# facebookresearch/rela

Hardware: AMD Instinct MI355X
Metric: env-steps/s (Ape-X Atari 84x84x4, actor tick + learner grad-step) (higher is better)
Workload: dtype f32 (f32 operands as 3 exact bf16 parts on bf16 MFMA; f32-accurate); 1 GPU; Ape-X DQN 80x80 envs/GPU, actor+learner on one MI355X, replay 2^20, B=512, A=18, n=3; device-resident static frames; parallelism=single

## Files before the change

### rela_amd/csrc/gemm_bf16x3.h

```cpp
#pragma once
#include <hip/hip_runtime.h>

#include <type_traits>

#include "common.h"
#include "gemm_lds.h"
#include "prof.h"

namespace rela_amd {
namespace gemm3 {

typedef float f32x4 __attribute__((ext_vector_type(4)));
typedef float f32x2 __attribute__((ext_vector_type(2)));
typedef __bf16 bf16x8 __attribute__((ext_vector_type(8)));
typedef __bf16 bf16x2 __attribute__((ext_vector_type(2)));
typedef short s16x4 __attribute__((ext_vector_type(4)));
typedef s16x4 __attribute__((address_space(3))) * lds_s16x4_ptr;

constexpr int kT = 512;
constexpr int BK = 32;

__device__ __forceinline__ int krow(int k) {
  const int g = k >> 3, j = k & 7;
  return j < 4 ? 4 * g + j : 16 + 4 * g + (j - 4);
}

__device__ __forceinline__ void split4(float4 v, uint2& hi, uint2& lo) {
  const f32x2 a = {v.x, v.y}, b = {v.z, v.w};
  const bf16x2 ha = __builtin_convertvector(a, bf16x2), hb = __builtin_convertvector(b, bf16x2);
  const bf16x2 la = __builtin_convertvector(a - __builtin_convertvector(ha, f32x2), bf16x2);
  const bf16x2 lb = __builtin_convertvector(b - __builtin_convertvector(hb, f32x2), bf16x2);
  hi = make_uint2(__builtin_bit_cast(uint32_t, ha), __builtin_bit_cast(uint32_t, hb));
  lo = make_uint2(__builtin_bit_cast(uint32_t, la), __builtin_bit_cast(uint32_t, lb));
}

__device__ __forceinline__ void split4x3(float4 v, uint2& hi, uint2& mid, uint2& lo) {
  const f32x2 a = {v.x, v.y}, b = {v.z, v.w};
  const bf16x2 ha = __builtin_convertvector(a, bf16x2), hb = __builtin_convertvector(b, bf16x2);
  const f32x2 ra = a - __builtin_convertvector(ha, f32x2), rb = b - __builtin_convertvector(hb, f32x2);
  const bf16x2 ma = __builtin_convertvector(ra, bf16x2), mb = __builtin_convertvector(rb, bf16x2);
  const bf16x2 la = __builtin_convertvector(ra - __builtin_convertvector(ma, f32x2), bf16x2);
  const bf16x2 lb = __builtin_convertvector(rb - __builtin_convertvector(mb, f32x2), bf16x2);
  hi = make_uint2(__builtin_bit_cast(uint32_t, ha), __builtin_bit_cast(uint32_t, hb));
  mid = make_uint2(__builtin_bit_cast(uint32_t, ma), __builtin_bit_cast(uint32_t, mb));
  lo = make_uint2(__builtin_bit_cast(uint32_t, la), __builtin_bit_cast(uint32_t, lb));
}

template <int BM_, int BN_, int WM_, int WN_, bool AMC_, int PARTS_ = 2>
struct TileCfg {
  static constexpr int BM = BM_, BN = BN_, WM = WM_, WN = WN_, PARTS = PARTS_;
  static constexpr bool AMC = AMC_;
  static_assert(PARTS == 2 || PARTS == 3, "two or three bf16 parts per operand");
  static_assert(WM * WN == 8, "8 wavefronts per block");
  static_assert(BM % 32 == 0 && BN % 32 == 0, "k-major row strides need multiples of 32 columns");
  static constexpr int TM = BM / 16 / WM, TN = BN / 16 / WN;
  static_assert(TM >= 1 && TN >= 1, "tile too small for the wave grid");
  static constexpr int LDA = AMC ? BM * 2 + 32 : BK * 2 + 16;
  static constexpr int A_HALF = AMC ? BK * LDA : BM * LDA;
  static constexpr int LDB = BN * 2 + 32;
  static constexpr int B_HALF = BK * LDB;
  static constexpr int BUF = PARTS * (A_HALF + B_HALF);
  static constexpr int LDS_BYTES = 2 * BUF;
  static constexpr int A_V4 = BM * BK / 4, B_V4 = BN * BK / 4;
  static constexpr int A_IT = (A_V4 + kT - 1) / kT, B_IT = (B_V4 + kT - 1) / kT;
};

struct GridMap {
  int gx, gy, gz;
  int mode;
};
__device__ __forceinline__ bool grid_map(const GridMap& gm, int& bx, int& by, int& bz) {
  if (gm.mode == 0) {
    bx = blockIdx.x, by = blockIdx.y, bz = blockIdx.z;
    return true;
  }
  const int xcd = blockIdx.x & 7, i = blockIdx.x >> 3;
  if (gm.mode == 1) {
    const int tiles = gm.gx * gm.gy;
    bz = (i / tiles) * 8 + xcd;
    const int t = i % tiles;
    bx = t % gm.gx, by = t / gm.gx;
    return bz < gm.gz;
  }
  bx = (i / gm.gy) * 8 + xcd, by = i % gm.gy, bz = 0;
  return bx < gm.gx;
}

template <class T, class P>
__global__ __launch_bounds__(kT) void gemm_bf16x3(const P p, const GridMap gm) {
  extern __shared__ __attribute__((aligned(16))) uint8_t smem[];
  int bx, by, bz;
  if (!grid_map(gm, bx, by, bz)) return;
  const int tid = threadIdx.x;
  const int wave = tid >> 6, lane = tid & 63;
  const int li = lane & 15, g = lane >> 4;
  const int wm = wave / T::WN, wn = wave % T::WN;
  const int m0 = by * T::BM, n0 = bx * T::BN;
  const int nch = (p.K + BK - 1) / BK;
  const int c0 = bz * p.kslice;
  const int c1 = min(nch, c0 + p.kslice);

  constexpr int D = 4;
  float4 ra[D][T::A_IT], rb[D][T::B_IT];
  auto gload = [&](int ch, auto set) {
    constexpr int S = decltype(set)::value;
    const int k0 = ch * BK;
#pragma unroll
    for (int j = 0; j < T::A_IT; ++j) {
      const int idx = min(tid + j * kT, T::A_V4 - 1);
      if constexpr (T::AMC) {
        const int kr = idx / (T::BM / 4), q = idx % (T::BM / 4);
        ra[S][j] = p.loadA(k0 + kr, m0 + 4 * q);
      } else {
        const int r = idx >> 3, q = idx & 7;
        ra[S][j] = p.loadA(m0 + r, k0 + 4 * q);
      }
    }
#pragma unroll
    for (int j = 0; j < T::B_IT; ++j) {
      const int idx = min(tid + j * kT, T::B_V4 - 1);
      const int kr = idx / (T::BN / 4), q = idx % (T::BN / 4);
      rb[S][j] = p.loadB(k0 + kr, n0 + 4 * q);
    }
  };
  auto sstore = [&](int buf, auto set) {
    constexpr int S = decltype(set)::value;
    uint8_t* base = smem + buf * T::BUF;
#pragma unroll
    for (int j = 0; j < T::A_IT; ++j) {
      const int idx = min(tid + j * kT, T::A_V4 - 1);
      uint2 hi, mid, lo;
      if constexpr (T::PARTS == 3) split4x3(ra[S][j], hi, mid, lo);
      else split4(ra[S][j], hi, lo);
      int off;
      if constexpr (T::AMC) {
        const int kr = idx / (T::BM / 4), q = idx % (T::BM / 4);
        off = krow(kr) * T::LDA + q * 8;
      } else {
        const int r = idx >> 3, q = idx & 7;
        off = r * T::LDA + q * 8;
      }
      *reinterpret_cast<uint2*>(base + off) = hi;
      if constexpr (T::PARTS == 3) *reinterpret_cast<uint2*>(base + T::A_HALF + off) = mid;
      *reinterpret_cast<uint2*>(base + (T::PARTS - 1) * T::A_HALF + off) = lo;
    }
    uint8_t* bb = base + T::PARTS * T::A_HALF;
#pragma unroll
    for (int j = 0; j < T::B_IT; ++j) {
      const int idx = min(tid + j * kT, T::B_V4 - 1);
      const int kr = idx / (T::BN / 4), q = idx % (T::BN / 4);
      uint2 hi, mid, lo;
      if constexpr (T::PARTS == 3) split4x3(rb[S][j], hi, mid, lo);
      else split4(rb[S][j], hi, lo);
      const int off = krow(kr) * T::LDB + q * 8;
      *reinterpret_cast<uint2*>(bb + off) = hi;
      if constexpr (T::PARTS == 3) *reinterpret_cast<uint2*>(bb + T::B_HALF + off) = mid;
      *reinterpret_cast<uint2*>(bb + (T::PARTS - 1) * T::B_HALF + off) = lo;
    }
  };

  const int tr_off = (4 * g + (li >> 2));
  auto frag_tr = [&](const uint8_t* img, int ld, int col0) -> bf16x8 {
    const uint8_t* a0 = img + tr_off * ld + (col0 + 4 * (li & 3)) * 2;
    const s16x4 x = __builtin_amdgcn_ds_read_tr16_b64_v4i16((lds_s16x4_ptr)(a0));
    const s16x4 y = __builtin_amdgcn_ds_read_tr16_b64_v4i16((lds_s16x4_ptr)(a0 + 16 * ld));
    typedef short s16x8 __attribute__((ext_vector_type(8)));
    const s16x8 z = {x[0], x[1], x[2], x[3], y[0], y[1], y[2], y[3]};
    return __builtin_bit_cast(bf16x8, z);
  };
  auto frag_row = [&](const uint8_t* img, int row) -> bf16x8 {
    return __builtin_bit_cast(bf16x8, *reinterpret_cast<const uint4*>(img + row * T::LDA + g * 16));
  };

  f32x4 acc[T::TM][T::TN];
  f32x4 accs[T::PARTS == 3 ? T::TM : 1][T::PARTS == 3 ? T::TN : 1];
#pragma unroll
  for (int t = 0; t < T::TM; ++t)
#pragma unroll
    for (int u = 0; u < T::TN; ++u) {
      acc[t][u] = f32x4{0.f, 0.f, 0.f, 0.f};
      if constexpr (T::PARTS == 3) accs[t][u] = f32x4{0.f, 0.f, 0.f, 0.f};
    }

  using S0 = std::integral_constant<int, 0>;
  using S1 = std::integral_constant<int, 1>;
  using S2 = std::integral_constant<int, 2>;
  using S3 = std::integral_constant<int, 3>;
  if (c0 < c1) gload(c0, S0{});
  if (c0 + 1 < c1) gload(c0 + 1, S1{});
  if (c0 + 2 < c1) gload(c0 + 2, S2{});
  if (c0 + 3 < c1) gload(c0 + 3, S3{});
  if (c0 < c1) sstore(0, S0{});
  __syncthreads();
  auto step = [&](int cur, auto cs, auto ns) {
    const int buf = (cur - c0) & 1;
    if (cur + D < c1) gload(cur + D, cs);
    const uint8_t* base = smem + buf * T::BUF;
    const uint8_t* bb = base + T::PARTS * T::A_HALF;
    bf16x8 bp[T::TN][T::PARTS];
#pragma unroll
    for (int u = 0; u < T::TN; ++u) {
      const int col0 = (wn * T::TN + u) * 16;
#pragma unroll
      for (int q = 0; q < T::PARTS; ++q) bp[u][q] = frag_tr(bb + q * T::B_HALF, T::LDB, col0);
    }
#pragma unroll
    for (int t = 0; t < T::TM; ++t) {
      const int row0 = (wm * T::TM + t) * 16;
      bf16x8 ap[T::PARTS];
#pragma unroll
      for (int q = 0; q < T::PARTS; ++q) {
        if constexpr (T::AMC) ap[q] = frag_tr(base + q * T::A_HALF, T::LDA, row0);
        else ap[q] = frag_row(base + q * T::A_HALF, row0 + li);
      }
#pragma unroll
      for (int u = 0; u < T::TN; ++u) {
        if constexpr (T::PARTS == 2) {
          acc[t][u] = __builtin_amdgcn_mfma_f32_16x16x32_bf16(ap[1], bp[u][0], acc[t][u], 0, 0, 0);
          acc[t][u] = __builtin_amdgcn_mfma_f32_16x16x32_bf16(ap[0], bp[u][1], acc[t][u], 0, 0, 0);
          acc[t][u] = __builtin_amdgcn_mfma_f32_16x16x32_bf16(ap[0], bp[u][0], acc[t][u], 0, 0, 0);
        } else {
          accs[t][u] = __builtin_amdgcn_mfma_f32_16x16x32_bf16(ap[2], bp[u][0], accs[t][u], 0, 0, 0);
          accs[t][u] = __builtin_amdgcn_mfma_f32_16x16x32_bf16(ap[0], bp[u][2], accs[t][u], 0, 0, 0);
          accs[t][u] = __builtin_amdgcn_mfma_f32_16x16x32_bf16(ap[1], bp[u][1], accs[t][u], 0, 0, 0);
          accs[t][u] = __builtin_amdgcn_mfma_f32_16x16x32_bf16(ap[1], bp[u][0], accs[t][u], 0, 0, 0);
          accs[t][u] = __builtin_amdgcn_mfma_f32_16x16x32_bf16(ap[0], bp[u][1], accs[t][u], 0, 0, 0);
          acc[t][u] = __builtin_amdgcn_mfma_f32_16x16x32_bf16(ap[0], bp[u][0], acc[t][u], 0, 0, 0);
        }
      }
    }
    if (cur + 1 < c1) sstore(buf ^ 1, ns);
    __syncthreads();
  };
  for (int base = c0; base < c1; base += D) {
    step(base, S0{}, S1{});
    if (base + 1 < c1) step(base + 1, S1{}, S2{});
    if (base + 2 < c1) step(base + 2, S2{}, S3{});
    if (base + 3 < c1) step(base + 3, S3{}, S0{});
  }

#pragma unroll
  for (int t = 0; t < T::TM; ++t)
#pragma unroll
    for (int u = 0; u < T::TN; ++u)
#pragma unroll
      for (int r = 0; r < 4; ++r) {
        const int m = m0 + (wm * T::TM + t) * 16 + g * 4 + r;
        const int n = n0 + (wn * T::TN + u) * 16 + li;
        if (m < p.M && n < p.N) {
          if constexpr (T::PARTS == 3) p.store(bz, m, n, acc[t][u][r] + accs[t][u][r]);
          else p.store(bz, m, n, acc[t][u][r]);
        }
      }
}

template <class T, class P>
int launch_gemm(P p, int splits, hipStream_t s, const char* name) {
  static const hipError_t attr_set = hipFuncSetAttribute(reinterpret_cast<const void*>(&gemm_bf16x3<T, P>),
                                                         hipFuncAttributeMaxDynamicSharedMemorySize, T::LDS_BYTES);
  RELA_HIP(attr_set);
  const int nch = ceil_div(p.K, BK);
  p.kslice = ceil_div(nch, splits);
  ProfScope prof(name, s);
  note_launch("gemm_bf16x3");
  constexpr bool xmap = true;
  GridMap gm{ceil_div(p.N, T::BN), ceil_div(p.M, T::BM), splits, 0};
  dim3 grid(gm.gx, gm.gy, gm.gz);
  if (xmap && gm.gz >= 8) {
    gm.mode = 1;
    grid = dim3(8 * gm.gx * gm.gy * ceil_div(gm.gz, 8));
  } else if (xmap && gm.gz == 1 && gm.gy > 1 && gm.gx >= 8) {
    gm.mode = 2;
    grid = dim3(8 * gm.gy * ceil_div(gm.gx, 8));
  }
  hipLaunchKernelGGL((gemm_bf16x3<T, P>), grid, dim3(kT), T::LDS_BYTES, s, p, gm);
  return RELA_OK;
}

}
}
```

### rela_amd/csrc/gemm_lds.h

```cpp
#pragma once
#include <hip/hip_runtime.h>

#include "common.h"
#include "prof.h"

namespace rela_amd {
namespace gemm {

typedef float f32x4 __attribute__((ext_vector_type(4)));
constexpr int kLT = 512;
constexpr int BK = 32;

__device__ __forceinline__ float4 zero4() { return make_float4(0.f, 0.f, 0.f, 0.f); }
__device__ __forceinline__ float4 ld4(const float* p) { return *reinterpret_cast<const float4*>(p); }

template <int BM_, int BN_, int WM_, int WN_, bool AMC_>
struct TileCfg {
  static constexpr int BM = BM_, BN = BN_, WM = WM_, WN = WN_;
  static constexpr bool AMC = AMC_;
  static_assert(WM * WN == 8, "8 wavefronts per block");
  static constexpr int TM = BM / 16 / WM, TN = BN / 16 / WN;
  static_assert(TM >= 1 && TN >= 1, "tile too small for the wave grid");
  static constexpr int LDA = AMC ? BM + 16 : BK + 2;
  static constexpr int A_FLOATS = AMC ? BK * LDA : BM * LDA;
  static constexpr int LDB = BN + 16;
  static constexpr int B_FLOATS = BK * LDB;
  static constexpr int A_V4 = BM * BK / 4, B_V4 = BN * BK / 4;
  static constexpr int A_IT = (A_V4 + kLT - 1) / kLT, B_IT = (B_V4 + kLT - 1) / kLT;
};

template <class T, class P>
__global__ __launch_bounds__(kLT) void gemm_lds(const P p) {
  __shared__ __attribute__((aligned(16))) float sA[2][T::A_FLOATS];
  __shared__ __attribute__((aligned(16))) float sB[2][T::B_FLOATS];
  const int tid = threadIdx.x;
  const int wave = tid >> 6, lane = tid & 63;
  const int li = lane & 15, kk = lane >> 4;
  const int wm = wave / T::WN, wn = wave % T::WN;
  const int m0 = blockIdx.y * T::BM, n0 = blockIdx.x * T::BN;
  const int nch = (p.K + BK - 1) / BK;
  const int c0 = blockIdx.z * p.kslice;
  const int c1 = min(nch, c0 + p.kslice);

  float4 ra[T::A_IT], rb[T::B_IT];
  auto gload = [&](int ch) {
    const int k0 = ch * BK;
#pragma unroll
    for (int j = 0; j < T::A_IT; ++j) {
      const int idx = tid + j * kLT;
      if (idx < T::A_V4) {
        if constexpr (T::AMC) {
          const int kr = idx / (T::BM / 4), q = idx % (T::BM / 4);
          ra[j] = p.loadA(k0 + kr, m0 + 4 * q);
        } else {
          const int r = idx >> 3, q = idx & 7;
          ra[j] = p.loadA(m0 + r, k0 + 4 * q);
        }
      }
    }
#pragma unroll
    for (int j = 0; j < T::B_IT; ++j) {
      const int idx = tid + j * kLT;
      if (idx < T::B_V4) {
        const int kr = idx / (T::BN / 4), q = idx % (T::BN / 4);
        rb[j] = p.loadB(k0 + kr, n0 + 4 * q);
      }
    }
  };
  auto sstore = [&](int buf) {
#pragma unroll
    for (int j = 0; j < T::A_IT; ++j) {
      const int idx = tid + j * kLT;
      if (idx < T::A_V4) {
        if constexpr (T::AMC) {
          const int kr = idx / (T::BM / 4), q = idx % (T::BM / 4);
          *reinterpret_cast<float4*>(&sA[buf][kr * T::LDA + 4 * q]) = ra[j];
        } else {
          const int r = idx >> 3, q = idx & 7;
          float* d = &sA[buf][r * T::LDA + 4 * q];
          *reinterpret_cast<float2*>(d) = make_float2(ra[j].x, ra[j].y);
          *reinterpret_cast<float2*>(d + 2) = make_float2(ra[j].z, ra[j].w);
        }
      }
    }
#pragma unroll
    for (int j = 0; j < T::B_IT; ++j) {
      const int idx = tid + j * kLT;
      if (idx < T::B_V4) {
        const int kr = idx / (T::BN / 4), q = idx % (T::BN / 4);
        *reinterpret_cast<float4*>(&sB[buf][kr * T::LDB + 4 * q]) = rb[j];
      }
    }
  };

  f32x4 acc[T::TM][T::TN];
#pragma unroll
  for (int t = 0; t < T::TM; ++t)
#pragma unroll
    for (int u = 0; u < T::TN; ++u) acc[t][u] = f32x4{0.f, 0.f, 0.f, 0.f};

  if (c0 < c1) {
    gload(c0);
    sstore(0);
  }
  __syncthreads();
  for (int ch = c0; ch < c1; ++ch) {
    const int buf = (ch - c0) & 1;
    if (ch + 1 < c1) gload(ch + 1);
#pragma unroll
    for (int ks = 0; ks < BK / 4; ++ks) {
      float a[T::TM], b[T::TN];
#pragma unroll
      for (int t = 0; t < T::TM; ++t) {
        const int row = (wm * T::TM + t) * 16 + li;
        a[t] = T::AMC ? sA[buf][(4 * ks + kk) * T::LDA + row] : sA[buf][row * T::LDA + 4 * ks + kk];
      }
#pragma unroll
      for (int u = 0; u < T::TN; ++u) b[u] = sB[buf][(4 * ks + kk) * T::LDB + (wn * T::TN + u) * 16 + li];
#pragma unroll
      for (int t = 0; t < T::TM; ++t)
#pragma unroll
        for (int u = 0; u < T::TN; ++u) acc[t][u] = __builtin_amdgcn_mfma_f32_16x16x4f32(a[t], b[u], acc[t][u], 0, 0, 0);
    }
    if (ch + 1 < c1) sstore(buf ^ 1);
    __syncthreads();
  }

#pragma unroll
  for (int t = 0; t < T::TM; ++t)
#pragma unroll
    for (int u = 0; u < T::TN; ++u)
#pragma unroll
      for (int r = 0; r < 4; ++r) {
        const int m = m0 + (wm * T::TM + t) * 16 + kk * 4 + r;
        const int n = n0 + (wn * T::TN + u) * 16 + li;
        if (m < p.M && n < p.N) p.store(blockIdx.z, m, n, acc[t][u][r]);
      }
}

struct ProbBase {
  int M, N, K, kslice;
};

template <class T, class P>
void launch_gemm(P p, int splits, hipStream_t s, const char* name) {
  const int nch = ceil_div(p.K, BK);
  p.kslice = ceil_div(nch, splits);
  ProfScope prof(name, s);
  note_launch("gemm_lds (f32)");
  hipLaunchKernelGGL((gemm_lds<T, P>), dim3(ceil_div(p.N, T::BN), ceil_div(p.M, T::BM), splits), dim3(kLT), 0, s, p);
}

}
}
```

### rela_amd/csrc/learner.hip

```cpp
#include "learner_common.h"

using namespace rela_amd;

struct rela_apex_learner {
  int device = 0;
  int A = 0, Bmax = 0;
  float gamma_n = 0.f;
  float vr_eps = 0.f;
  bool loss_called = false;
  int optimizer = 0;
  float lr = 0.f, opt_eps = 0.f, clip = 0.f;
  int64_t adam_t = 0;
  int64_t off[13] = {0};
  float *P = nullptr, *PT = nullptr, *G = nullptr, *S1 = nullptr, *S2 = nullptr;
  rela_ffnet *online = nullptr, *target = nullptr;
  float *w2p = nullptr, *w3p = nullptr, *wfcp = nullptr;
  void *ws_on = nullptr, *ws_tmp = nullptr;
  int64_t ws_bytes = 0;
  float *q = nullptr;
  float *td = nullptr, *d_ha = nullptr, *d_h = nullptr, *d_a3 = nullptr, *d_a2 = nullptr, *d_a1 = nullptr;
  float *col = nullptr;
  float *part = nullptr;
  float *cpart = nullptr;
  float *s32 = nullptr;
  double* npart = nullptr;
  float* norm = nullptr;
  float* loss = nullptr;
  bool loaded = false;
  int pend_B = 0, last_B = 0;
  int pend_rows = 0;
  const uint8_t* pend_obs = nullptr;
  hipStream_t side = nullptr;
  hipEvent_t ev[8] = {nullptr};
  float *part_side = nullptr, *cpart_side = nullptr;
  void *frag2 = nullptr, *frag3 = nullptr;
};

namespace {
rela_ffnet_params params_at(const rela_apex_learner* l, float* base) {
  rela_ffnet_params p;
  const float** f = reinterpret_cast<const float**>(&p);
  for (int i = 0; i < 12; ++i) f[i] = base + l->off[i];
  return p;
}

int repack(rela_apex_learner* l, bool online, bool target, hipStream_t s) {
  if (online) {
    const rela_ffnet_params p = params_at(l, l->P);
    FFNetExtraPacks extra;
    extra.w2p = l->w2p, extra.w3p = l->w3p, extra.wfcp = l->wfcp;
    int rc = ffnet_load_extra(l->online, &p, s, extra);
    if (rc != RELA_OK) return rc;
    if (l->frag2) dgfast::pack_frags(l->w2p, l->w3p, l->frag2, l->frag3, s);
  }
  if (target) {
    const rela_ffnet_params p = params_at(l, l->PT);
    int rc = rela_ffnet_load(l->target, &p, 1, s);
    if (rc != RELA_OK) return rc;
  }
  return RELA_OK;
}
}

extern "C" int rela_apex_learner_create(rela_apex_learner** out, int num_action, int max_batch, int multi_step,
                                        float gamma, int optimizer, float lr, float eps, float grad_clip,
                                        int device) {
  RELA_CHECK(out && num_action >= 1 && num_action <= 31 && max_batch >= 1 && multi_step >= 1 &&
                 (optimizer == 0 || optimizer == 1),
             RELA_EINVAL, "rela_apex_learner_create: bad arguments (A=%d batch=%d n=%d optimizer=%d)", num_action,
             max_batch, multi_step, optimizer);
  int ndev = 0;
  if (hipGetDeviceCount(&ndev) != hipSuccess || device < 0 || device >= ndev) {
    set_last_error("rela_apex_learner_create: HIP device %d not available (%d visible); there is no CPU path",
                   device, ndev);
    return RELA_ENODEV;
  }
  DeviceGuard g(device);
  auto* l = new rela_apex_learner();
  l->device = device;
  l->A = num_action;
  l->Bmax = max_batch;
  l->gamma_n = (float)pow((double)gamma, (double)multi_step);
  l->optimizer = optimizer;
  l->lr = lr;
  l->opt_eps = eps;
  l->clip = grad_clip;
  const int64_t cnt[12] = {32 * 256, 32, 64 * 512, 64, 64 * 576, 64, (int64_t)512 * 3136, 512, 512, 1,
                           (int64_t)num_action * 512, num_action};
  for (int i = 0; i < 12; ++i) l->off[i + 1] = l->off[i] + (cnt[i] + 3) / 4 * 4;
  const size_t nb = sizeof(float) * (size_t)l->off[12];
  const size_t B = (size_t)max_batch, A = (size_t)num_action;
  RELA_HIP(hipMalloc(&l->P, nb));
  RELA_HIP(hipMalloc(&l->PT, nb));
  RELA_HIP(hipMalloc(&l->G, nb));
  RELA_HIP(hipMalloc(&l->S1, nb));
  RELA_HIP(hipMalloc(&l->S2, nb));
  RELA_HIP(hipMemset(l->P, 0, nb));
  RELA_HIP(hipMemset(l->PT, 0, nb));
  RELA_HIP(hipMemset(l->G, 0, nb));
  RELA_HIP(hipMemset(l->S1, 0, nb));
  RELA_HIP(hipMemset(l->S2, 0, nb));
  int rc = rela_ffnet_create(&l->online, num_action, device);
  if (rc != RELA_OK) return rc;
  rc = rela_ffnet_create(&l->target, num_action, device);
  if (rc != RELA_OK) return rc;
  ffnet_label_as_learner(l->online);
  ffnet_label_as_learner(l->target);
  ffnet_set_max_rows(l->online, max_batch);
  ffnet_set_max_rows(l->target, max_batch);
  RELA_HIP(hipMalloc(&l->w2p, sizeof(float) * 64 * 512));
  RELA_HIP(hipMalloc(&l->w3p, sizeof(float) * 64 * 576));
  RELA_HIP(hipMalloc(&l->wfcp, sizeof(float) * 512 * 3136));
  l->ws_bytes = std::max(rela_ffnet_workspace_bytes(nullptr, max_batch), rela_ffnet_workspace_bytes(nullptr, 2 * max_batch));
  RELA_HIP(hipMalloc(&l->ws_on, (size_t)l->ws_bytes));
  RELA_HIP(hipMalloc(&l->ws_tmp, (size_t)l->ws_bytes));
  RELA_HIP(hipMalloc(&l->q, sizeof(float) * 3 * B * A));
  RELA_HIP(hipMalloc(&l->td, sizeof(float) * B));
  RELA_HIP(hipMalloc(&l->d_ha, sizeof(float) * B * 32));
  RELA_HIP(hipMalloc(&l->d_h, sizeof(float) * B * 512));
  RELA_HIP(hipMalloc(&l->d_a3, sizeof(float) * B * kA3));
  RELA_HIP(hipMalloc(&l->d_a2, sizeof(float) * B * kA2));
  RELA_HIP(hipMalloc(&l->d_a1, sizeof(float) * B * kA1));
  RELA_HIP(hipMalloc(&l->col, sizeof(float) * trunk_col_floats(B)));
  RELA_HIP(hipMalloc(&l->part, sizeof(float) * kTrunkPartFloats));
  RELA_HIP(hipMalloc(&l->cpart, sizeof(float) * kColsumBlocks * (32 + 512 + 64 + 64 + 32)));
  RELA_HIP(hipMalloc(&l->s32, sizeof(float) * 32));
  RELA_HIP(hipMalloc(&l->npart, sizeof(double) * kNormBlocks));
  RELA_HIP(hipMalloc(&l->norm, sizeof(float) * 2));
  RELA_HIP(hipMalloc(&l->loss, sizeof(float)));
  static const bool lanes = !(getenv("RELA_LEARNER_LANES") && atoi(getenv("RELA_LEARNER_LANES")) == 1);
  if (lanes) {
    RELA_HIP(hipStreamCreateWithFlags(&l->side, hipStreamNonBlocking));
    for (hipEvent_t& e : l->ev) RELA_HIP(hipEventCreateWithFlags(&e, hipEventDisableTiming));
    RELA_HIP(hipMalloc(&l->part_side, sizeof(float) * kTrunkPartFloats));
    RELA_HIP(hipMalloc(&l->cpart_side, sizeof(float) * kColsumBlocks * (32 + 512 + 64 + 64 + 32)));
    RELA_HIP(hipMalloc(&l->frag2, dgfast::kFrag2Bytes));
    RELA_HIP(hipMalloc(&l->frag3, dgfast::kFrag3Bytes));
  }
  *out = l;
  return RELA_OK;
}

extern "C" void rela_apex_learner_destroy(rela_apex_learner* l) {
  if (!l) return;
  DeviceGuard g(l->device);
  (void)hipDeviceSynchronize();
  void* ps[] = {l->P,  l->PT,   l->G,    l->S1,   l->S2,   l->w2p, l->w3p,  l->wfcp,  l->ws_on, l->ws_tmp, l->q,
                l->td, l->d_ha, l->d_h,  l->d_a3, l->d_a2, l->d_a1, l->col, l->part,  l->cpart, l->s32,    l->npart,
                l->norm, l->loss, l->part_side, l->cpart_side, l->frag2, l->frag3};
  for (void* p : ps) (void)hipFree(p);
  for (hipEvent_t e : l->ev)
    if (e) (void)hipEventDestroy(e);
  if (l->side) (void)hipStreamDestroy(l->side);
  rela_ffnet_destroy(l->online);
  rela_ffnet_destroy(l->target);
  delete l;
}

extern "C" int rela_apex_learner_load(rela_apex_learner* l, const rela_ffnet_params* online,
                                      const rela_ffnet_params* target, int on_device, void* stream_) {
  RELA_CHECK(l && online, RELA_EINVAL, "rela_apex_learner_load: bad arguments");
  hipStream_t s = (hipStream_t)stream_;
  DeviceGuard g(l->device);
  const hipMemcpyKind kind = on_device ? hipMemcpyDeviceToDevice : hipMemcpyHostToDevice;
  const float* const* fo = reinterpret_cast<const float* const*>(online);
  const float* const* ft = reinterpret_cast<const float* const*>(target ? target : online);
  const int64_t cnt[12] = {32 * 256, 32, 64 * 512, 64, 64 * 576, 64, (int64_t)512 * 3136, 512, 512, 1,
                           (int64_t)l->A * 512, l->A};
  for (int i = 0; i < 12; ++i) {
    RELA_CHECK(fo[i] && ft[i], RELA_EINVAL, "rela_apex_learner_load: parameter %d is NULL", i);
    RELA_HIP(hipMemcpyAsync(l->P + l->off[i], fo[i], sizeof(float) * cnt[i], kind, s));
    RELA_HIP(hipMemcpyAsync(l->PT + l->off[i], ft[i], sizeof(float) * cnt[i], kind, s));
  }
  if (!on_device) RELA_HIP(hipStreamSynchronize(s));
  const size_t nb = sizeof(float) * (size_t)l->off[12];
  RELA_HIP(hipMemsetAsync(l->S1, 0, nb, s));
  RELA_HIP(hipMemsetAsync(l->S2, 0, nb, s));
  l->adam_t = 0;
  int rc = repack(l, true, true, s);
  if (rc != RELA_OK) return rc;
  l->loaded = true;
  return RELA_OK;
}

extern "C" int rela_apex_learner_set_value_rescale(rela_apex_learner* l, float eps) {
  RELA_CHECK(l && eps == eps, RELA_EINVAL, "rela_apex_learner_set_value_rescale: bad arguments");
  RELA_CHECK(!l->loss_called, RELA_ESTATE, "rela_apex_learner_set_value_rescale: call it before the first loss");
  l->vr_eps = eps > 0.f ? eps : 0.f;
  return RELA_OK;
}

extern "C" int rela_apex_learner_set_precision(rela_apex_learner* l, int mode) {
  RELA_CHECK(l && mode >= 0 && mode <= 2, RELA_EINVAL, "rela_apex_learner_set_precision: mode must be 0, 1 or 2");
  int rc = rela_ffnet_set_precision(l->online, mode);
  if (rc != RELA_OK) return rc;
  return rela_ffnet_set_precision(l->target, mode);
}

extern "C" int rela_apex_learner_sync_target(rela_apex_learner* l, void* stream_) {
  RELA_CHECK(l && l->loaded, RELA_ESTATE, "rela_apex_learner_sync_target: parameters were never loaded");
  hipStream_t s = (hipStream_t)stream_;
  DeviceGuard g(l->device);
  RELA_HIP(hipMemcpyAsync(l->PT, l->P, sizeof(float) * (size_t)l->off[12], hipMemcpyDeviceToDevice, s));
  return repack(l, false, true, s);
}

extern "C" int rela_apex_learner_params(rela_apex_learner* l, rela_ffnet_params* online_out,
                                        rela_ffnet_params* target_out) {
  RELA_CHECK(l, RELA_EINVAL, "rela_apex_learner_params: bad arguments");
  if (online_out) *online_out = params_at(l, l->P);
  if (target_out) *target_out = params_at(l, l->PT);
  return RELA_OK;
}

extern "C" int rela_apex_learner_grads(rela_apex_learner* l, rela_ffnet_params* grads_out) {
  RELA_CHECK(l && grads_out, RELA_EINVAL, "rela_apex_learner_grads: bad arguments");
  *grads_out = params_at(l, l->G);
  return RELA_OK;
}

extern "C" int rela_apex_learner_flat(rela_apex_learner* l, float** params_dev, float** grads_dev, int64_t* count) {
  RELA_CHECK(l, RELA_EINVAL, "rela_apex_learner_flat: bad arguments");
  if (params_dev) *params_dev = l->P;
  if (grads_dev) *grads_dev = l->G;
  if (count) *count = l->off[12];
  return RELA_OK;
}

extern "C" const float* rela_apex_learner_stats_dev(const rela_apex_learner* l) { return l ? l->norm : nullptr; }

extern "C" int rela_apex_learner_debug_activations(rela_apex_learner* l, float** a1, float** a2, float** a3, float** h,
                                                   int* batch) {
  RELA_CHECK(l && l->last_B > 0, RELA_ESTATE, "rela_apex_learner_debug_activations: no rela_apex_learner_loss yet");
  const FFNetWs w = ffnet_ws(l->ws_on, l->pend_rows);
  if (a1) *a1 = w.a1;
  if (a2) *a2 = w.a2;
  if (a3) *a3 = w.a3;
  if (h) *h = w.h;
  if (batch) *batch = l->last_B;
  return RELA_OK;
}

extern "C" int rela_apex_learner_backward(rela_apex_learner* l, int batch, const void* const* rows_dev,
                                          const float* weight_dev, float* priority_dev, float* loss_dev,
                                          void* stream_) {
  int rc = rela_apex_learner_loss(l, batch, rows_dev, weight_dev, priority_dev, loss_dev, stream_);
  if (rc != RELA_OK) return rc;
  return rela_apex_learner_grad(l, stream_);
}

static bool merge_online_forwards() {
  static const bool on = [] {
    const char* e = getenv("RELA_LEARNER_MERGE_ONLINE");
    return !(e && e[0] == '0');
  }();
  return on;
}

extern "C" int rela_apex_learner_loss(rela_apex_learner* l, int batch, const void* const* rows_dev,
                                      const float* weight_dev, float* priority_dev, float* loss_dev, void* stream_) {
  RELA_CHECK(l && l->loaded, RELA_ESTATE, "rela_apex_learner_loss: parameters were never loaded");
  RELA_CHECK(batch >= 1 && batch <= l->Bmax && rows_dev && weight_dev && priority_dev, RELA_EINVAL,
             "rela_apex_learner_loss: bad arguments (batch %d, max %d)", batch, l->Bmax);
  l->pend_B = 0;
  l->loss_called = true;
  hipStream_t s = (hipStream_t)stream_;
  DeviceGuard g(l->device);
  const int Bn = batch, A = l->A;
  const uint8_t* obs = static_cast<const uint8_t*>(rows_dev[0]);
  const uint8_t* nobs = static_cast<const uint8_t*>(rows_dev[1]);
  const float* legal = static_cast<const float*>(rows_dev[4]);
  const float* nlegal = static_cast<const float*>(rows_dev[5]);
  const int64_t* act = static_cast<const int64_t*>(rows_dev[6]);
  const float* reward = static_cast<const float*>(rows_dev[7]);
  const float* boot = static_cast<const float*>(rows_dev[9]);
  RELA_CHECK(obs && nobs && legal && nlegal && act && reward && boot, RELA_EINVAL,
             "rela_apex_learner_loss: a batch field is NULL");
  float* q_on = l->q;
  float* q_no = l->q + (size_t)Bn * A;
  float* q_nt = l->q + 2 * (size_t)Bn * A;
  int rc;
  bool unsplit_side = false;
  l->pend_rows = Bn;
  if (rela_ffnet_precision(l->online) == 1 && ffnet_learner_forward_ok(l->online, l->target, Bn)) {
    rc = ffnet_learner_forward(l->online, l->target, Bn, obs, nobs, legal, nlegal, q_on, q_no, q_nt, l->ws_on, l->ws_tmp,
                               l->ws_bytes, s);
    if (rc != RELA_OK) return rc;
    if (l->side) lane_dep(l->ev[0], s, l->side);
    rc = ffnet_learner_unsplit(Bn, l->ws_on, l->side ? l->side : s);
    if (rc != RELA_OK) return rc;
    unsplit_side = l->side != nullptr;
    l->pend_rows = 2 * Bn;
  } else if (rela_ffnet_precision(l->online) == 2 && Bn >= 512 && merge_online_forwards() &&
             nobs == obs + (size_t)Bn * 28224 && nlegal == legal + (size_t)Bn * A) {
    const uint8_t* in2 = obs;
    const float* legal2 = legal;
    rc = rela_ffnet_forward(l->target, Bn, nobs, nlegal, q_nt, l->ws_tmp, l->ws_bytes, s);
    if (rc != RELA_OK) return rc;
    ffnet_set_max_rows(l->online, 2 * l->Bmax);
    rc = ffnet_forward_mode(l->online, 2 * Bn, in2, legal2, q_on, l->ws_on, l->ws_bytes, s, 3);
    ffnet_set_max_rows(l->online, l->Bmax);
    if (rc != RELA_OK) return rc;
    l->pend_rows = 2 * Bn;
  } else {
    rc = rela_ffnet_forward(l->online, Bn, nobs, nlegal, q_no, l->ws_tmp, l->ws_bytes, s);
    if (rc != RELA_OK) return rc;
    rc = rela_ffnet_forward(l->target, Bn, nobs, nlegal, q_nt, l->ws_tmp, l->ws_bytes, s);
    if (rc != RELA_OK) return rc;
    rc = ffnet_forward_mode(l->online, Bn, obs, legal, q_on, l->ws_on, l->ws_bytes, s, rela_ffnet_precision(l->online) == 2 ? 3 : 0);
    if (rc != RELA_OK) return rc;
  }
  if (Bn <= 1024) {
    ProfScope prof("learner_loss_grad", s);
    hipLaunchKernelGGL(learner_td_loss_grad, dim3(1), dim3(1024), 0, s, Bn, A, (const float*)q_on, (const float*)q_no,
                       (const float*)q_nt, nlegal, act, reward, boot, l->gamma_n, l->vr_eps, weight_dev, legal, l->td,
                       priority_dev, l->d_ha, l->loss);
  } else {
    rc = td_from_q(Bn, A, 0, q_on, q_no, q_nt, nlegal, act, reward, boot, l->gamma_n, l->vr_eps, l->td, priority_dev, s);
    if (rc != RELA_OK) return rc;
    ProfScope prof("learner_loss_grad", s);
    hipLaunchKernelGGL(learner_loss_grad, dim3(1), dim3(kLT), 0, s, (const float*)l->td, weight_dev, act, legal, Bn,
                       A, l->d_ha, l->loss);
  }
  if (loss_dev) RELA_HIP(dev_copy2(loss_dev, l->loss, sizeof(float), nullptr, nullptr, 0, s));
  if (unsplit_side) lane_dep(l->ev[1], l->side, s);
  RELA_LAUNCH_CHECK();
  l->pend_B = l->last_B = Bn;
  l->pend_obs = obs;
  return RELA_OK;
}

extern "C" int rela_apex_learner_grad(rela_apex_learner* l, void* stream_) {
  RELA_CHECK(l && l->loaded && l->pend_B > 0, RELA_ESTATE, "rela_apex_learner_grad: no rela_apex_learner_loss to differentiate");
  hipStream_t s = (hipStream_t)stream_;
  DeviceGuard g(l->device);
  const int Bn = l->pend_B, A = l->A;
  const uint8_t* obs = l->pend_obs;
  l->pend_B = 0;

  const FFNetWs w = ffnet_ws(l->ws_on, l->pend_rows);
  const rela_ffnet_params P = params_at(l, l->P);
  float* Gm[12];
  for (int i = 0; i < 12; ++i) Gm[i] = l->G + l->off[i];

  ColsumJobs sums;
  const bool g3 = rela_ffnet_precision(l->online) == 1 && gemm_bf16x3_on();
  const bool g6 = rela_ffnet_precision(l->online) == 2;
  const bool lanes = l->side != nullptr;
  hipStream_t sw = lanes ? l->side : s;
  if (lanes) lane_dep(l->ev[2], s, sw);

  {
    ProbHeadDgrad p{};
    p.M = Bn, p.N = 512, p.K = 32;
    p.d_ha = l->d_ha, p.a_w = P.a_w, p.v_w = P.v_w, p.h = w.h, p.d_h = l->d_h, p.A = A;
    if (g3) (void)gemm3::launch_gemm<Tile3Dgrad>(p, 1, s, "learner_dgrad_heads");
    else if (g6) (void)gemm3::launch_gemm<Tile6Dgrad>(p, 1, s, "learner_dgrad_heads");
    else launch_gemm<TileDgrad>(p, 1, s, "learner_dgrad_heads");
  }
  {
    ProbHeadWgrad p{};
    p.M = 32, p.N = 512, p.K = Bn;
    p.d_ha = l->d_ha, p.h = w.h, p.g_a_w = Gm[10], p.g_v_w = Gm[8], p.A = A;
    if (g3) (void)gemm3::launch_gemm<Tile3W32>(p, 1, sw, "learner_wgrad_heads");
    else if (g6) (void)gemm3::launch_gemm<Tile6W32>(p, 1, sw, "learner_wgrad_heads");
    else launch_gemm<TileW32>(p, 1, sw, "learner_wgrad_heads");
  }
  sums.add(l->d_ha, Bn, 32, l->s32);
  if (lanes) lane_dep(l->ev[3], s, sw);
  {
    ProbFcDgrad p{};
    p.M = Bn, p.N = 3136, p.K = 512;
    p.d_h = l->d_h, p.wfcp = l->wfcp, p.a3 = w.a3, p.d_a3 = l->d_a3;
    if (g3) (void)gemm3::launch_gemm<Tile3Dgrad>(p, 1, s, "learner_dgrad_fc");
    else if (g6) (void)gemm3::launch_gemm<Tile6Dgrad>(p, 1, s, "learner_dgrad_fc");
    else launch_gemm<TileDgrad>(p, 1, s, "learner_dgrad_fc");
  }
  {
    ProbFcWgrad p{};
    p.M = 512, p.N = 3136, p.K = Bn;
    p.d_h = l->d_h, p.a3 = w.a3, p.g_fc_w = Gm[6];
    if (g3) (void)gemm3::launch_gemm<Tile3Wfc>(p, 1, sw, "learner_wgrad_fc");
    else if (g6) (void)gemm3::launch_gemm<Tile6Wfc>(p, 1, sw, "learner_wgrad_fc");
    else launch_gemm<TileWfc>(p, 1, sw, "learner_wgrad_fc");
  }
  sums.add(l->d_h, Bn, 512, Gm[7]);
  {
    TrunkBwd t{};
    t.Bn = Bn, t.obs = obs, t.a1 = w.a1, t.a2 = w.a2, t.d_a3 = l->d_a3, t.d_a2 = l->d_a2, t.d_a1 = l->d_a1;
    t.col = l->col, t.part = l->part, t.cpart = l->cpart, t.w2p = l->w2p, t.w3p = l->w3p;
    t.g_c1w = Gm[0], t.g_c1b = Gm[1], t.g_c2w = Gm[2], t.g_c2b = Gm[3], t.g_c3w = Gm[4], t.g_c3b = Gm[5];
    t.fast = rela_ffnet_precision(l->online) == 1;
    t.emu = g6;
    if (lanes) {
      t.side = sw, t.ev_da3 = l->ev[4], t.ev_da2 = l->ev[5], t.ev_side = l->ev[6];
      t.part_side = l->part_side, t.cpart_side = l->cpart_side;
      if (t.fast) t.frag2 = l->frag2, t.frag3 = l->frag3;
      t.s32 = l->s32, t.A = A, t.g_a_b = Gm[11], t.g_v_b = Gm[9];
    }
    trunk_backward(t, s, &sums);
    if (!lanes) hipLaunchKernelGGL(head_bias_grad, dim3(1), dim3(32), 0, s, (const float*)l->s32, A, Gm[11], Gm[9]);
  }
  RELA_LAUNCH_CHECK();
  return RELA_OK;
}

namespace {
struct TrunkTapScratch {
  std::vector<void*> bufs;
  hipStream_t side = nullptr;
  hipEvent_t ev[3] = {nullptr, nullptr, nullptr};
  ~TrunkTapScratch() {
    for (void* p : bufs) (void)hipFree(p);
    for (hipEvent_t e : ev)
      if (e) (void)hipEventDestroy(e);
    if (side) (void)hipStreamDestroy(side);
  }
  template <class T>
  hipError_t alloc(T** p, size_t bytes) {
    void* v = nullptr;
    const hipError_t e = hipMalloc(&v, bytes);
    if (e == hipSuccess) bufs.push_back(v);
    *p = static_cast<T*>(v);
    return e;
  }
};
}

extern "C" int rela_debug_trunk_backward(int frames, int mode, int lanes, int fast_wgrad_min_frames, const uint8_t* obs,
                                         const float* a1, const float* a2, const float* d_a3, const float* conv2_w,
                                         const float* conv3_w, float* g_c1w, float* g_c1b, float* g_c2w, float* g_c2b,
                                         float* g_c3w, float* g_c3b, float* d_a2, float* d_a1, void* stream_) {
  RELA_CHECK(frames >= 1 && frames <= 65536 && mode >= 0 && mode <= 2 && (lanes == 0 || lanes == 1), RELA_EINVAL,
             "rela_debug_trunk_backward: bad arguments (frames %d, mode %d, lanes %d)", frames, mode, lanes);
  RELA_CHECK(obs && a1 && a2 && d_a3 && conv2_w && conv3_w && g_c1w && g_c1b && g_c2w && g_c2b && g_c3w && g_c3b && d_a2 &&
                 d_a1,
             RELA_EINVAL, "rela_debug_trunk_backward: a pointer is NULL");
  hipStream_t s = (hipStream_t)stream_;
  TrunkTapScratch sc;
  const size_t cpart_bytes = sizeof(float) * kColsumBlocks * (32 + 512 + 64 + 64 + 32);
  float *w2p = nullptr, *w3p = nullptr;
  RELA_HIP(sc.alloc(&w2p, sizeof(float) * 64 * 512));
  RELA_HIP(sc.alloc(&w3p, sizeof(float) * 64 * 576));
  hipLaunchKernelGGL(permute_weights, dim3(ceil_div(64 * 512, 256)), dim3(256), 0, s, kPermConv2, conv2_w, w2p, 64 * 512);
  hipLaunchKernelGGL(permute_weights, dim3(ceil_div(64 * 576, 256)), dim3(256), 0, s, kPermConv3, conv3_w, w3p, 64 * 576);
  TrunkBwd t{};
  t.Bn = frames, t.obs = obs, t.a1 = a1, t.a2 = a2, t.d_a3 = d_a3, t.d_a2 = d_a2, t.d_a1 = d_a1;
  t.w2p = w2p, t.w3p = w3p;
  t.g_c1w = g_c1w, t.g_c1b = g_c1b, t.g_c2w = g_c2w, t.g_c2b = g_c2b, t.g_c3w = g_c3w, t.g_c3b = g_c3b;
  t.fast = mode == 1;
  if (fast_wgrad_min_frames > 0) t.fast_wgrad_min_frames = fast_wgrad_min_frames;
  RELA_HIP(sc.alloc(&t.col, sizeof(float) * trunk_col_floats((size_t)frames)));
  RELA_HIP(sc.alloc(&t.part, sizeof(float) * kTrunkPartFloats));
  RELA_HIP(sc.alloc(&t.cpart, cpart_bytes));
  t.emu = mode == 2;
  if (lanes) {
    RELA_HIP(hipStreamCreateWithFlags(&sc.side, hipStreamNonBlocking));
    for (hipEvent_t& e : sc.ev) RELA_HIP(hipEventCreateWithFlags(&e, hipEventDisableTiming));
    t.side = sc.side, t.ev_da3 = sc.ev[0], t.ev_da2 = sc.ev[1], t.ev_side = sc.ev[2];
    RELA_HIP(sc.alloc(&t.part_side, sizeof(float) * kTrunkPartFloats));
    RELA_HIP(sc.alloc(&t.cpart_side, cpart_bytes));
    if (t.fast) {
      void *frag2 = nullptr, *frag3 = nullptr;
      RELA_HIP(sc.alloc(&frag2, dgfast::kFrag2Bytes));
      RELA_HIP(sc.alloc(&frag3, dgfast::kFrag3Bytes));
      dgfast::pack_frags(w2p, w3p, frag2, frag3, s);
      t.frag2 = frag2, t.frag3 = frag3;
    }
  }
  trunk_backward(t, s);
  const hipError_t launched = hipGetLastError();
  const hipError_t done = hipStreamSynchronize(s);
  if (sc.side) (void)hipStreamSynchronize(sc.side);
  RELA_HIP(launched);
  RELA_HIP(done);
  return RELA_OK;
}

extern "C" int rela_apex_learner_apply(rela_apex_learner* l, void* stream_) {
  RELA_CHECK(l && l->loaded, RELA_ESTATE, "rela_apex_learner_apply: parameters were never loaded");
  hipStream_t s = (hipStream_t)stream_;
  DeviceGuard g(l->device);
  OptimState o;
  o.optimizer = l->optimizer, o.lr = l->lr, o.eps = l->opt_eps, o.clip = l->clip, o.adam_t = l->adam_t;
  optimizer_apply(o, l->P, l->G, l->S1, l->S2, l->off[12], l->npart, l->norm, s);
  l->adam_t = o.adam_t;
  RELA_LAUNCH_CHECK();
  return repack(l, true, false, s);
}
```

### rela_amd/csrc/learner_common.h

```cpp
#pragma once
#include <cmath>
#include <cstring>
#include <vector>

#include "common.h"
#include "ffnet_layout.h"
#include "gemm_lds.h"
#include "gemm_bf16x3.h"
#include "prof.h"
#include "value_rescale.h"
#include "dgrad_conv_bf16.h"
#include "wgrad_conv1_bf16.h"
#include "wgrad_conv2_bf16.h"
#include "wgrad_conv3_bf16.h"

namespace rela_amd {
namespace {

using namespace gemm;

using TileDgrad = TileCfg<128, 64, 4, 2, false>;
using TileWfc = TileCfg<128, 64, 4, 2, true>;
using TileW64 = TileCfg<64, 64, 2, 4, true>;
using TileW32 = TileCfg<32, 64, 2, 4, true>;
using Tile3Dgrad = gemm3::TileCfg<128, 64, 4, 2, false>;
using Tile3Wfc = gemm3::TileCfg<128, 64, 4, 2, true>;
using Tile3W64 = gemm3::TileCfg<64, 64, 2, 4, true>;
using Tile3W32 = gemm3::TileCfg<32, 64, 2, 4, true>;
inline bool gemm_bf16x3_on() { return true; }
using Tile6Dgrad = gemm3::TileCfg<128, 64, 4, 2, false, 3>;
using Tile6Wfc = gemm3::TileCfg<128, 64, 4, 2, true, 3>;
using Tile6W64 = gemm3::TileCfg<64, 64, 2, 4, true, 3>;
using Tile6W32 = gemm3::TileCfg<32, 64, 2, 4, true, 3>;


struct ProbHeadDgrad : ProbBase {
  const float *d_ha, *a_w, *v_w, *h;
  float* d_h;
  int A;
  __device__ float4 loadA(int m, int k) const { return m < M ? ld4(d_ha + (size_t)m * 32 + k) : zero4(); }
  __device__ float4 loadB(int k, int n) const {
    if (k < A) return ld4(a_w + (size_t)k * 512 + n);
    if (k == 31) return ld4(v_w + n);
    return zero4();
  }
  __device__ void store(int, int m, int n, float v) const {
    const size_t i = (size_t)m * 512 + n;
    d_h[i] = h[i] > 0.f ? v : 0.f;
  }
};

struct ProbHeadWgradPart : ProbBase {
  const float *d_ha, *h;
  float* part;
  __device__ float4 loadA(int b, int m) const { return b < K ? ld4(d_ha + (size_t)b * 32 + m) : zero4(); }
  __device__ float4 loadB(int b, int n) const { return b < K ? ld4(h + (size_t)b * 512 + n) : zero4(); }
  __device__ void store(int z, int m, int n, float v) const { part[((size_t)z * 32 + m) * 512 + n] = v; }
};
__global__ void head_wgrad_reduce(const float* __restrict__ part, int splits, int A, float* __restrict__ g_a_w,
                                  float* __restrict__ g_v_w) {
  const int idx = blockIdx.x * blockDim.x + threadIdx.x;
  if (idx >= 32 * 512) return;
  const int m = idx >> 9, n = idx & 511;
  if (m >= A && m != 31) return;
  float s = 0.f;
#pragma unroll 8
  for (int z = 0; z < splits; ++z) s += part[(size_t)z * (32 * 512) + idx];
  if (m < A) g_a_w[(size_t)m * 512 + n] = s;
  else g_v_w[n] = s;
}

struct ProbHeadWgrad : ProbBase {
  const float *d_ha, *h;
  float *g_a_w, *g_v_w;
  int A;
  __device__ float4 loadA(int b, int m) const { return b < K ? ld4(d_ha + (size_t)b * 32 + m) : zero4(); }
  __device__ float4 loadB(int b, int n) const { return b < K ? ld4(h + (size_t)b * 512 + n) : zero4(); }
  __device__ void store(int, int m, int n, float v) const {
    if (m < A) g_a_w[(size_t)m * 512 + n] = v;
    else if (m == 31) g_v_w[n] = v;
  }
};

struct ProbFcDgrad : ProbBase {
  const float *d_h, *wfcp, *a3;
  float* d_a3;
  __device__ float4 loadA(int m, int k) const { return m < M ? ld4(d_h + (size_t)m * 512 + k) : zero4(); }
  __device__ float4 loadB(int k, int n) const { return ld4(wfcp + (size_t)k * 3136 + n); }
  __device__ void store(int, int m, int n, float v) const {
    const size_t i = (size_t)m * 3136 + n;
    d_a3[i] = a3[i] > 0.f ? v : 0.f;
  }
};

struct ProbFcWgrad : ProbBase {
  const float *d_h, *a3;
  float* g_fc_w;
  __device__ float4 loadA(int b, int m) const { return b < K ? ld4(d_h + (size_t)b * 512 + m) : zero4(); }
  __device__ float4 loadB(int b, int n) const { return b < K ? ld4(a3 + (size_t)b * 3136 + n) : zero4(); }
  __device__ void store(int, int m, int n, float v) const {
    const int pos = n >> 6, c = n & 63;
    g_fc_w[(size_t)m * 3136 + c * 49 + pos] = v;
  }
};

struct ProbConvDgrad : ProbBase {
  const float *d_out, *wp;
  float* col;
  __device__ float4 loadA(int m, int k) const { return m < M ? ld4(d_out + (size_t)m * 64 + k) : zero4(); }
  __device__ float4 loadB(int k, int n) const { return ld4(wp + (size_t)k * N + n); }
  __device__ void store(int, int m, int n, float v) const { col[(size_t)m * N + n] = v; }
};

template <int OC, int CIN, int KH, int KW, int STRIDE, int OH, int OW, int IH, int IW>
struct ProbConvWgrad : ProbBase {
  const float *d_out, *in;
  float* part;
  __device__ float4 loadA(int k, int m) const { return k < K ? ld4(d_out + (size_t)k * OC + m) : zero4(); }
  __device__ float4 loadB(int k, int n) const {
    if (k >= K) return zero4();
    const int b = k / (OH * OW), pos = k - b * (OH * OW);
    const int oy = pos / OW, ox = pos - oy * OW;
    const int r = n / CIN, c = n - r * CIN;
    const int kh = r / KW, kw = r - kh * KW;
    return ld4(in + (((size_t)b * IH + oy * STRIDE + kh) * IW + ox * STRIDE + kw) * CIN + c);
  }
  __device__ void store(int z, int m, int n, float v) const { part[((size_t)z * M + m) * N + n] = v; }
};
using ProbW3 = ProbConvWgrad<64, 64, 3, 3, 1, 7, 7, 9, 9>;
using ProbW2 = ProbConvWgrad<64, 32, 4, 4, 2, 9, 9, 20, 20>;

struct ProbW1 : ProbBase {
  const float* d_out;
  const uint8_t* obs;
  float* part;
  __device__ float4 loadA(int k, int m) const { return k < K ? ld4(d_out + (size_t)k * 32 + m) : zero4(); }
  __device__ float4 loadB(int k, int n) const {
    if (k >= K) return zero4();
    const int b = k / 400, pos = k - b * 400;
    const int oy = pos / 20, ox = pos - oy * 20;
    const int c = n >> 6, kh = (n >> 3) & 7, kw = n & 7;
    const uint32_t d = *reinterpret_cast<const uint32_t*>(obs + (size_t)b * 28224 + c * 7056 + (oy * 4 + kh) * 84 +
                                                          ox * 4 + kw);
    return make_float4((float)(d & 0xff), (float)((d >> 8) & 0xff), (float)((d >> 16) & 0xff), (float)(d >> 24));
  }
  __device__ void store(int z, int m, int n, float v) const { part[((size_t)z * M + m) * N + n] = v; }
};


__global__ void col2im3(const float* __restrict__ col, const float* __restrict__ a2, float* __restrict__ d_a2,
                        int Bn) {
  const int idx = blockIdx.x * blockDim.x + threadIdx.x;
  if (idx >= Bn * 81 * 16) return;
  const int c4 = idx & 15, pix = idx >> 4;
  const int x = pix % 9, y = (pix / 9) % 9, b = pix / 81;
  float4 s = zero4();
  for (int kh = 0; kh < 3; ++kh) {
    const int oy = y - kh;
    if (oy < 0 || oy >= 7) continue;
    for (int kw = 0; kw < 3; ++kw) {
      const int ox = x - kw;
      if (ox < 0 || ox >= 7) continue;
      const float4 v = ld4(col + ((size_t)b * 49 + oy * 7 + ox) * 576 + (kh * 3 + kw) * 64 + c4 * 4);
      s.x += v.x, s.y += v.y, s.z += v.z, s.w += v.w;
    }
  }
  const float4 a = ld4(a2 + (size_t)pix * 64 + c4 * 4);
  *reinterpret_cast<float4*>(d_a2 + (size_t)pix * 64 + c4 * 4) =
      make_float4(a.x > 0.f ? s.x : 0.f, a.y > 0.f ? s.y : 0.f, a.z > 0.f ? s.z : 0.f, a.w > 0.f ? s.w : 0.f);
}

__global__ void col2im2(const float* __restrict__ col, const float* __restrict__ a1, float* __restrict__ d_a1,
                        int Bn) {
  const int idx = blockIdx.x * blockDim.x + threadIdx.x;
  if (idx >= Bn * 400 * 8) return;
  const int c4 = idx & 7, pix = idx >> 3;
  const int x = pix % 20, y = (pix / 20) % 20, b = pix / 400;
  float4 s = zero4();
  for (int kh = 0; kh < 4; ++kh) {
    const int ty = y - kh;
    if (ty < 0 || (ty & 1) || ty > 16) continue;
    for (int kw = 0; kw < 4; ++kw) {
      const int tx = x - kw;
      if (tx < 0 || (tx & 1) || tx > 16) continue;
      const float4 v = ld4(col + ((size_t)b * 81 + (ty >> 1) * 9 + (tx >> 1)) * 512 + (kh * 4 + kw) * 32 + c4 * 4);
      s.x += v.x, s.y += v.y, s.z += v.z, s.w += v.w;
    }
  }
  const float4 a = ld4(a1 + (size_t)pix * 32 + c4 * 4);
  *reinterpret_cast<float4*>(d_a1 + (size_t)pix * 32 + c4 * 4) =
      make_float4(a.x > 0.f ? s.x : 0.f, a.y > 0.f ? s.y : 0.f, a.z > 0.f ? s.z : 0.f, a.w > 0.f ? s.w : 0.f);
}

enum { kRedConv1 = 0, kRedConv2 = 1, kRedConv3 = 2 };
__global__ void reduce_splits(const float* __restrict__ part, int splits, int M, int N, int mode,
                              float* __restrict__ out) {
  const int idx = blockIdx.x * blockDim.x + threadIdx.x;
  if (idx >= M * N) return;
  const int m = idx / N, n = idx - m * N;
  float s = 0.f;
#pragma unroll 8
  for (int z = 0; z < splits; ++z) s += part[((size_t)z * M + m) * N + n];
  if (mode == kRedConv1) {
    out[(size_t)m * N + n] = s / 255.0f;
  } else if (mode == kRedConv2) {
    const int c = n & 31, r = n >> 5;
    out[((size_t)(m * 32 + c) * 4 + (r >> 2)) * 4 + (r & 3)] = s;
  } else {
    const int c = n & 63, r = n >> 6;
    out[((size_t)(m * 64 + c) * 3 + r / 3) * 3 + r % 3] = s;
  }
}

constexpr int kColsumBlocks = 256;
__global__ __launch_bounds__(kLT) void colsum_partial(const float* __restrict__ src, int64_t rows, int C,
                                                      float* __restrict__ part) {
  __shared__ float4 sm[kLT];
  const int G = C / 4, L = kLT / G;
  const int cg = threadIdx.x % G, rl = threadIdx.x / G;
  const int64_t per = (rows + gridDim.x - 1) / gridDim.x;
  const int64_t r0 = blockIdx.x * per, r1 = min(rows, r0 + per);
  float4 s = zero4();
  for (int64_t r = r0 + rl; r < r1; r += L) {
    const float4 v = ld4(src + r * C + cg * 4);
    s.x += v.x, s.y += v.y, s.z += v.z, s.w += v.w;
  }
  sm[threadIdx.x] = s;
  __syncthreads();
  if (rl == 0) {
    for (int l = 1; l < L; ++l) {
      const float4 v = sm[cg + l * G];
      s.x += v.x, s.y += v.y, s.z += v.z, s.w += v.w;
    }
    *reinterpret_cast<float4*>(part + (size_t)blockIdx.x * C + cg * 4) = s;
  }
}
__global__ __launch_bounds__(kColsumBlocks) void colsum_final(const float* __restrict__ part, int C,
                                                              float* __restrict__ out) {
  __shared__ float4 sm[kColsumBlocks];
  const int cg = blockIdx.x;
  sm[threadIdx.x] = ld4(part + (size_t)threadIdx.x * C + cg * 4);
  __syncthreads();
  for (int o = kColsumBlocks / 2; o > 0; o >>= 1) {
    if ((int)threadIdx.x < o) {
      const float4 v = sm[threadIdx.x + o];
      float4& d = sm[threadIdx.x];
      d.x += v.x, d.y += v.y, d.z += v.z, d.w += v.w;
    }
    __syncthreads();
  }
  if (threadIdx.x == 0) *reinterpret_cast<float4*>(out + cg * 4) = sm[0];
}
constexpr int kMaxColsumJobs = 6;
struct ColsumJobs {
  const float* src[kMaxColsumJobs];
  float* out[kMaxColsumJobs];
  float* part[kMaxColsumJobs];
  int64_t rows[kMaxColsumJobs];
  int C[kMaxColsumJobs];
  int n = 0;
  void add(const float* s, int64_t r, int c, float* o) { src[n] = s, rows[n] = r, C[n] = c, out[n] = o, ++n; }
};
__global__ __launch_bounds__(kLT) void colsum_partial_multi(ColsumJobs jobs) {
  __shared__ float4 sm[kLT];
  const int j = blockIdx.y;
  const float* src = jobs.src[j];
  const int64_t rows = jobs.rows[j];
  const int C = jobs.C[j];
  const int G = C / 4, L = kLT / G;
  const int cg = threadIdx.x % G, rl = threadIdx.x / G;
  const int64_t per = (rows + gridDim.x - 1) / gridDim.x;
  const int64_t r0 = blockIdx.x * per, r1 = min(rows, r0 + per);
  float4 s = zero4();
  int64_t r = r0 + rl;
  for (; r + 7 * (int64_t)L < r1; r += 8 * (int64_t)L) {
    float4 v[8];
#pragma unroll
    for (int u = 0; u < 8; ++u) v[u] = ld4(src + (r + u * (int64_t)L) * C + cg * 4);
#pragma unroll
    for (int u = 0; u < 8; ++u) s.x += v[u].x, s.y += v[u].y, s.z += v[u].z, s.w += v[u].w;
  }
  for (; r < r1; r += L) {
    const float4 v = ld4(src + r * C + cg * 4);
    s.x += v.x, s.y += v.y, s.z += v.z, s.w += v.w;
  }
  sm[threadIdx.x] = s;
  __syncthreads();
  if (rl == 0) {
    for (int l = 1; l < L; ++l) {
      const float4 v = sm[cg + l * G];
      s.x += v.x, s.y += v.y, s.z += v.z, s.w += v.w;
    }
    *reinterpret_cast<float4*>(jobs.part[j] + (size_t)blockIdx.x * C + cg * 4) = s;
  }
}
__global__ __launch_bounds__(kColsumBlocks) void colsum_final_multi(ColsumJobs jobs) {
  __shared__ float4 sm[kColsumBlocks];
  const int j = blockIdx.y, cg = blockIdx.x, C = jobs.C[j];
  if (cg >= C / 4) return;
  sm[threadIdx.x] = ld4(jobs.part[j] + (size_t)threadIdx.x * C + cg * 4);
  __syncthreads();
  for (int o = kColsumBlocks / 2; o > 0; o >>= 1) {
    if ((int)threadIdx.x < o) {
      const float4 v = sm[threadIdx.x + o];
      float4& d = sm[threadIdx.x];
      d.x += v.x, d.y += v.y, d.z += v.z, d.w += v.w;
    }
    __syncthreads();
  }
  if (threadIdx.x == 0) *reinterpret_cast<float4*>(jobs.out[j] + cg * 4) = sm[0];
}
__global__ void head_bias_grad(const float* __restrict__ s32, int A, float* __restrict__ g_a_b,
                               float* __restrict__ g_v_b) {
  const int k = threadIdx.x;
  if (k < A) g_a_b[k] = s32[k];
  if (k == 31) g_v_b[0] = s32[31];
}

__global__ __launch_bounds__(kLT) void learner_loss_grad(const float* __restrict__ td, const float* __restrict__ w,
                                                         const int64_t* __restrict__ act,
                                                         const float* __restrict__ legal, int Bn, int A,
                                                         float* __restrict__ d_ha, float* __restrict__ loss_out) {
  __shared__ float red[kLT];
  float lsum = 0.f;
  const float inv_b = 1.0f / (float)Bn, inv_a = 1.0f / (float)A;
  for (int i = threadIdx.x; i < Bn; i += kLT) {
    const float e = td[i], ae = fabsf(e);
    lsum += (ae < 1.0f ? 0.5f * e * e : ae - 0.5f) * w[i];
    const float g = -(w[i] * fminf(fmaxf(e, -1.0f), 1.0f)) * inv_b;
    const int a = (int)act[i];
    float* row = d_ha + (size_t)i * 32;
    for (int k = 0; k < 32; ++k) {
      float v = 0.f;
      if (k < A) v = legal[(size_t)i * A + k] * (g * ((k == a ? 1.0f : 0.0f) - inv_a));
      if (k == 31) v = g;
      row[k] = v;
    }
  }
  red[threadIdx.x] = lsum;
  __syncthreads();
  for (int o = kLT / 2; o > 0; o >>= 1) {
    if (threadIdx.x < o) red[threadIdx.x] += red[threadIdx.x + o];
    __syncthreads();
  }
  if (threadIdx.x == 0) loss_out[0] = red[0] * inv_b;
}

__global__ __launch_bounds__(1024) void learner_td_loss_grad(int Bn, int A, const float* __restrict__ q,
                                                             const float* __restrict__ qno, const float* __restrict__ qnt,
                                                             const float* __restrict__ nlegal,
                                                             const int64_t* __restrict__ act,
                                                             const float* __restrict__ reward,
                                                             const float* __restrict__ bootstrap, float gamma_n,
                                                             float vr_eps, const float* __restrict__ w,
                                                             const float* __restrict__ legal,
                                                             float* __restrict__ td, float* __restrict__ prio,
                                                             float* __restrict__ d_ha, float* __restrict__ loss_out) {
  __shared__ float red[1024];
  float m = INFINITY;
  for (int i = threadIdx.x; i < Bn * A; i += 1024) m = fminf(m, qno[i]);
  red[threadIdx.x] = m;
  __syncthreads();
  for (int off = 512; off > 0; off >>= 1) {
    if ((int)threadIdx.x < off) red[threadIdx.x] = fminf(red[threadIdx.x], red[threadIdx.x + off]);
    __syncthreads();
  }
  const float qmin = red[0];
  __syncthreads();
  float lsum = 0.f;
  const float inv_b = 1.0f / (float)Bn, inv_a = 1.0f / (float)A;
  for (int i = threadIdx.x; i < Bn; i += 1024) {
    int na = 0;
    float bv = -INFINITY;
#pragma unroll 6
    for (int j = 0; j < A; ++j) {
      const float lq = __fmul_rn(__fsub_rn(__fadd_rn(1.0f, qno[(size_t)i * A + j]), qmin), nlegal[(size_t)i * A + j]);
      if (lq > bv) bv = lq, na = j;
    }
    const int a = (int)act[i];
    const float qa = q[(size_t)i * A + a];
    const float bq = qnt[(size_t)i * A + na];
    float tgt;
    if (vr_eps > 0.0f)
      tgt = rela_vr::h(__fadd_rn(reward[i], __fmul_rn(__fmul_rn(bootstrap[i], gamma_n), rela_vr::h_inv(bq, vr_eps))), vr_eps);
    else
      tgt = __fadd_rn(reward[i], __fmul_rn(__fmul_rn(bootstrap[i], gamma_n), bq));
    const float e = __fsub_rn(tgt, qa), ae = fabsf(e);
    td[i] = e;
    prio[i] = ae;
    lsum += (ae < 1.0f ? 0.5f * e * e : ae - 0.5f) * w[i];
    const float g = -(w[i] * fminf(fmaxf(e, -1.0f), 1.0f)) * inv_b;
    float4* row = reinterpret_cast<float4*>(d_ha + (size_t)i * 32);
    float v[32];
#pragma unroll
    for (int k = 0; k < 32; ++k) {
      v[k] = 0.f;
      if (k < A) v[k] = legal[(size_t)i * A + k] * (g * ((k == a ? 1.0f : 0.0f) - inv_a));
      if (k == 31) v[k] = g;
    }
#pragma unroll
    for (int k = 0; k < 8; ++k) row[k] = make_float4(v[4 * k], v[4 * k + 1], v[4 * k + 2], v[4 * k + 3]);
  }
  red[threadIdx.x] = lsum;
  __syncthreads();
  for (int o = 512; o > 0; o >>= 1) {
    if ((int)threadIdx.x < o) red[threadIdx.x] += red[threadIdx.x + o];
    __syncthreads();
  }
  if (threadIdx.x == 0) loss_out[0] = red[0] * inv_b;
}

__global__ void permute_weights(int mode, const float* __restrict__ src, float* __restrict__ dst, int total) {
  const int idx = blockIdx.x * blockDim.x + threadIdx.x;
  if (idx < total) permute_weight_at(mode, idx, src, dst);
}

constexpr int kNormBlocks = 256;
__global__ __launch_bounds__(256) void sumsq_partial(const float* __restrict__ g, int64_t n, double* __restrict__ part) {
  __shared__ double red[256];
  double s = 0.0;
  const int64_t n4 = n >> 2, stride = (int64_t)gridDim.x * 256;
  const float4* g4 = reinterpret_cast<const float4*>(g);
  int64_t i = (int64_t)blockIdx.x * 256 + threadIdx.x;
  for (; i + 3 * stride < n4; i += 4 * stride) {
    float4 v[4];
#pragma unroll
    for (int u = 0; u < 4; ++u) v[u] = g4[i + u * stride];
#pragma unroll
    for (int u = 0; u < 4; ++u)
      s += (double)v[u].x * (double)v[u].x + (double)v[u].y * (double)v[u].y + (double)v[u].z * (double)v[u].z +
           (double)v[u].w * (double)v[u].w;
  }
  for (; i < n4; i += stride) {
    const float4 v = g4[i];
    s += (double)v.x * (double)v.x + (double)v.y * (double)v.y + (double)v.z * (double)v.z + (double)v.w * (double)v.w;
  }
  if (blockIdx.x == 0 && threadIdx.x < (n & 3)) s += (double)g[(n4 << 2) + threadIdx.x] * (double)g[(n4 << 2) + threadIdx.x];
  red[threadIdx.x] = s;
  __syncthreads();
  for (int o = 128; o > 0; o >>= 1) {
    if (threadIdx.x < o) red[threadIdx.x] += red[threadIdx.x + o];
    __syncthreads();
  }
  if (threadIdx.x == 0) part[blockIdx.x] = red[0];
}
__global__ __launch_bounds__(256) void clip_coef(const double* __restrict__ part, int nblk, float max_norm,
                                                 float* __restrict__ out, const unsigned* __restrict__ abort_word) {
  __shared__ double red[256];
  red[threadIdx.x] = (int)threadIdx.x < nblk ? part[threadIdx.x] : 0.0;
  __syncthreads();
  for (int o = 128; o > 0; o >>= 1) {
    if ((int)threadIdx.x < o) red[threadIdx.x] += red[threadIdx.x + o];
    __syncthreads();
  }
  if (threadIdx.x != 0) return;
  const double s = red[0];
  const float norm = (float)sqrt(s);
  out[0] = norm;
  const float c = max_norm / (norm + 1e-6f);
  out[1] = c < 1.0f ? c : 1.0f;
  if (abort_word && *abort_word != 0) out[1] = -1.0f;
}
__global__ void rmsprop_update(float* __restrict__ p, const float* __restrict__ g, float* __restrict__ sq, int64_t n4,
                               float lr, float alpha, float eps, const float* __restrict__ coef) {
  const int64_t i = (int64_t)blockIdx.x * blockDim.x + threadIdx.x;
  const float cf = coef[1];
  if (i >= n4 || cf < 0.f) return;
  const float4 gv = reinterpret_cast<const float4*>(g)[i];
  float4 sv = reinterpret_cast<float4*>(sq)[i], pv = reinterpret_cast<float4*>(p)[i];
  auto upd = [&](float gi, float& s, float& pi) {
    gi = gi * cf;
    s = alpha * s + (1.0f - alpha) * gi * gi;
    pi -= lr * (gi / (sqrtf(s) + eps));
  };
  upd(gv.x, sv.x, pv.x), upd(gv.y, sv.y, pv.y), upd(gv.z, sv.z, pv.z), upd(gv.w, sv.w, pv.w);
  reinterpret_cast<float4*>(sq)[i] = sv;
  reinterpret_cast<float4*>(p)[i] = pv;
}
__global__ void adam_update(float* __restrict__ p, const float* __restrict__ g, float* __restrict__ m1,
                            float* __restrict__ m2, int64_t n4, float lr, float b1, float b2, float eps, float bc1,
                            float bc2_sqrt, const float* __restrict__ coef) {
  const int64_t i = (int64_t)blockIdx.x * blockDim.x + threadIdx.x;
  const float cf = coef[1];
  if (i >= n4 || cf < 0.f) return;
  const float4 gv = reinterpret_cast<const float4*>(g)[i];
  float4 av = reinterpret_cast<float4*>(m1)[i], bv = reinterpret_cast<float4*>(m2)[i], pv = reinterpret_cast<float4*>(p)[i];
  auto upd = [&](float gi, float& a, float& b, float& pi) {
    gi = gi * cf;
    a = b1 * a + (1.0f - b1) * gi;
    b = b2 * b + (1.0f - b2) * gi * gi;
    pi -= (lr / bc1) * (a / (sqrtf(b) / bc2_sqrt + eps));
  };
  upd(gv.x, av.x, bv.x, pv.x), upd(gv.y, av.y, bv.y, pv.y), upd(gv.z, av.z, bv.z, pv.z), upd(gv.w, av.w, bv.w, pv.w);
  reinterpret_cast<float4*>(m1)[i] = av;
  reinterpret_cast<float4*>(m2)[i] = bv;
  reinterpret_cast<float4*>(p)[i] = pv;
}


constexpr int kSplitW3 = 28, kSplitW2 = 27, kSplitW1 = 64;
constexpr size_t kTrunkPartFloats = (size_t)w3fast::kMaxBlocks * 64 * 576;
static_assert(kTrunkPartFloats * 4 >= dgfast::kFrag3Bytes && kTrunkPartFloats * 4 >= dgfast::kFrag2Bytes, "frag scratch");
static_assert(kTrunkPartFloats >= (size_t)kSplitW3 * 8 * 64 * 576, "part size (split multiplier up to 8)");
static_assert(kTrunkPartFloats >= (size_t)kSplitW3 * 64 * 576 && kTrunkPartFloats >= (size_t)w1fast::kMaxBlocks * 32 * 256 &&
                  kTrunkPartFloats >= (size_t)w2fast::kMaxBlocks * 64 * 512,
              "part size");
static_assert(kSplitW3 * 64 * 576 >= kSplitW2 * 64 * 512 && kSplitW3 * 64 * 576 >= kSplitW1 * 32 * 256, "part size");
inline size_t trunk_col_floats(size_t frames) { return frames * (size_t)(81 * 512 > 49 * 576 ? 81 * 512 : 49 * 576); }

constexpr int kFastWgradMinFrames = 2048;
struct TrunkBwd {
  int Bn;
  const uint8_t* obs;
  const float *a1, *a2;
  const float* d_a3;
  float *d_a2, *d_a1;
  float* col;
  float* part;
  float* cpart;
  const float *w2p, *w3p;
  float *g_c1w, *g_c1b, *g_c2w, *g_c2b, *g_c3w, *g_c3b;
  bool fast = false;
  bool emu = false;
  int fast_wgrad_min_frames = kFastWgradMinFrames;
  hipStream_t side = nullptr;
  hipEvent_t ev_da3 = nullptr, ev_da2 = nullptr, ev_side = nullptr;
  float *part_side = nullptr, *cpart_side = nullptr;
  const void *frag2 = nullptr, *frag3 = nullptr;
  const float* s32 = nullptr;
  float *g_a_b = nullptr, *g_v_b = nullptr;
  int A = 0;
};
inline void lane_dep(hipEvent_t ev, hipStream_t from, hipStream_t to) {
  (void)hipEventRecord(ev, from);
  (void)hipStreamWaitEvent(to, ev, 0);
}

inline void colsum_multi_launch(ColsumJobs& jobs, float* cpart, hipStream_t s) {
  if (jobs.n == 0) return;
  int maxC = 0;
  size_t off = 0;
  for (int j = 0; j < jobs.n; ++j) {
    jobs.part[j] = cpart + off;
    off += (size_t)kColsumBlocks * jobs.C[j];
    maxC = jobs.C[j] > maxC ? jobs.C[j] : maxC;
  }
  ProfScope prof("learner_colsum", s);
  hipLaunchKernelGGL(colsum_partial_multi, dim3(kColsumBlocks, jobs.n), dim3(kLT), 0, s, jobs);
  hipLaunchKernelGGL(colsum_final_multi, dim3(maxC / 4, jobs.n), dim3(kColsumBlocks), 0, s, jobs);
}

inline void colsum_launch(const float* src, int64_t rows, int C, float* cpart, float* out, hipStream_t s) {
  ProfScope prof("learner_colsum", s);
  hipLaunchKernelGGL(colsum_partial, dim3(kColsumBlocks), dim3(kLT), 0, s, src, rows, C, cpart);
  hipLaunchKernelGGL(colsum_final, dim3(C / 4), dim3(kColsumBlocks), 0, s, (const float*)cpart, C, out);
}

inline void trunk_backward(const TrunkBwd& t, hipStream_t s, ColsumJobs* pending = nullptr) {
  const int Bn = t.Bn;
  ColsumJobs own;
  ColsumJobs& jobs = pending ? *pending : own;
  const bool lanes = t.side != nullptr;
  hipStream_t sw = lanes ? t.side : s;
  float* partw = lanes ? t.part_side : t.part;
  if (lanes) lane_dep(t.ev_da3, s, sw);
  const bool fast23 = t.fast && Bn >= t.fast_wgrad_min_frames;
  if (fast23) {
    int blocks = 0;
    {
      ProfScope prof("learner_wgrad_conv3", sw);
      (void)w3fast::launch(t.a2, t.d_a3, Bn, partw, sw, &blocks);
    }
    hipLaunchKernelGGL(reduce_splits, dim3(ceil_div(64 * 576, 256)), dim3(256), 0, sw, (const float*)partw, blocks, 64,
                       576, kRedConv3, t.g_c3w);
  } else {
    ProbW3 p{};
    p.M = 64, p.N = 576, p.K = Bn * 49;
    p.d_out = t.d_a3, p.in = t.a2, p.part = partw;
    static const int mul = 3  ;
    const int split3 = Bn <= 1024 ? kSplitW3 * mul : kSplitW3;
    if (t.fast && gemm_bf16x3_on()) (void)gemm3::launch_gemm<Tile3W64>(p, split3, sw, "learner_wgrad_conv3");
    else if (t.emu) (void)gemm3::launch_gemm<Tile6W64>(p, split3, sw, "learner_wgrad_conv3");
    else launch_gemm<TileW64>(p, split3, sw, "learner_wgrad_conv3");
    hipLaunchKernelGGL(reduce_splits, dim3(ceil_div(64 * 576, 256)), dim3(256), 0, sw, (const float*)partw, split3, 64,
                       576, kRedConv3, t.g_c3w);
  }
  jobs.add(t.d_a3, (int64_t)Bn * 49, 64, t.g_c3b);
  if (t.fast) {
    ProfScope prof("learner_dgrad_conv3", s);
    (void)dgfast::launch_conv3(t.d_a3, t.w3p, t.a2, t.d_a2, Bn, t.part, s, t.frag3);
  } else {
    ProbConvDgrad p{};
    p.M = Bn * 49, p.N = 576, p.K = 64;
    p.d_out = t.d_a3, p.wp = t.w3p, p.col = t.col;
    launch_gemm<TileDgrad>(p, 1, s, "learner_dgrad_conv3");
    ProfScope prof("learner_col2im", s);
    hipLaunchKernelGGL(col2im3, dim3(ceil_div((int64_t)Bn * 81 * 16, 256)), dim3(256), 0, s, (const float*)t.col, t.a2,
                       t.d_a2, Bn);
  }
  if (lanes) lane_dep(t.ev_da2, s, sw);
  if (fast23) {
    int blocks = 0;
    {
      ProfScope prof("learner_wgrad_conv2", sw);
      (void)w2fast::launch(t.a1, t.d_a2, Bn, partw, sw, &blocks);
    }
    hipLaunchKernelGGL(reduce_splits, dim3(ceil_div(64 * 512, 256)), dim3(256), 0, sw, (const float*)partw, blocks, 64,
                       512, kRedConv2, t.g_c2w);
  } else {
    ProbW2 p{};
    p.M = 64, p.N = 512, p.K = Bn * 81;
    p.d_out = t.d_a2, p.in = t.a1, p.part = partw;
    static const int mul = 3  ;
    const int split2 = Bn <= 1024 ? kSplitW2 * mul : kSplitW2;
    if (t.fast && gemm_bf16x3_on()) (void)gemm3::launch_gemm<Tile3W64>(p, split2, sw, "learner_wgrad_conv2");
    else if (t.emu) (void)gemm3::launch_gemm<Tile6W64>(p, split2, sw, "learner_wgrad_conv2");
    else launch_gemm<TileW64>(p, split2, sw, "learner_wgrad_conv2");
    hipLaunchKernelGGL(reduce_splits, dim3(ceil_div(64 * 512, 256)), dim3(256), 0, sw, (const float*)partw, split2, 64,
                       512, kRedConv2, t.g_c2w);
  }
  jobs.add(t.d_a2, (int64_t)Bn * 81, 64, t.g_c2b);
  if (lanes) {
    colsum_multi_launch(jobs, t.cpart_side, sw);
    if (t.s32) hipLaunchKernelGGL(head_bias_grad, dim3(1), dim3(32), 0, sw, t.s32, t.A, t.g_a_b, t.g_v_b);
    jobs.n = 0;
  }
  if (t.fast) {
    ProfScope prof("learner_dgrad_conv2", s);
    (void)dgfast::launch_conv2(t.d_a2, t.w2p, t.a1, t.d_a1, Bn, t.part, s, t.frag2);
  } else {
    ProbConvDgrad p{};
    p.M = Bn * 81, p.N = 512, p.K = 64;
    p.d_out = t.d_a2, p.wp = t.w2p, p.col = t.col;
    launch_gemm<TileDgrad>(p, 1, s, "learner_dgrad_conv2");
    ProfScope prof("learner_col2im", s);
    hipLaunchKernelGGL(col2im2, dim3(ceil_div((int64_t)Bn * 400 * 8, 256)), dim3(256), 0, s, (const float*)t.col, t.a1,
                       t.d_a1, Bn);
  }
  if (t.fast) {
    int blocks = 0;
    {
      ProfScope prof("learner_wgrad_conv1", s);
      (void)w1fast::launch(t.obs, t.d_a1, Bn, t.part, s, &blocks, lanes ? 128 : w1fast::kMaxBlocks);
    }
    hipLaunchKernelGGL(reduce_splits, dim3(ceil_div(32 * 256, 256)), dim3(256), 0, s, (const float*)t.part, blocks, 32,
                       256, kRedConv1, t.g_c1w);
  } else {
    ProbW1 p{};
    p.M = 32, p.N = 256, p.K = Bn * 400;
    p.d_out = t.d_a1, p.obs = t.obs, p.part = t.part;
    if (t.emu) (void)gemm3::launch_gemm<Tile6W32>(p, kSplitW1, s, "learner_wgrad_conv1");
    else launch_gemm<TileW32>(p, kSplitW1, s, "learner_wgrad_conv1");
    hipLaunchKernelGGL(reduce_splits, dim3(ceil_div(32 * 256, 256)), dim3(256), 0, s, (const float*)t.part, kSplitW1, 32,
                       256, kRedConv1, t.g_c1w);
  }
  jobs.add(t.d_a1, (int64_t)Bn * 400, 32, t.g_c1b);
  colsum_multi_launch(jobs, t.cpart, s);
  if (lanes) lane_dep(t.ev_side, sw, s);
}

struct OptimState {
  int optimizer = 0;
  float lr = 0.f, eps = 0.f, clip = 0.f;
  int64_t adam_t = 0;
};
inline void optimizer_apply(OptimState& o, float* P, const float* G, float* S1, float* S2, int64_t n, double* npart,
                            float* norm, hipStream_t s, const unsigned* abort_word = nullptr) {
  ProfScope prof("learner_optimizer", s);
  hipLaunchKernelGGL(sumsq_partial, dim3(kNormBlocks), dim3(256), 0, s, G, n, npart);
  hipLaunchKernelGGL(clip_coef, dim3(1), dim3(256), 0, s, (const double*)npart, kNormBlocks, o.clip, norm, abort_word);
  if (o.optimizer == 0) {
    hipLaunchKernelGGL(rmsprop_update, dim3(ceil_div(n / 4, 256)), dim3(256), 0, s, P, G, S1, n / 4, o.lr, 0.99f, o.eps,
                       (const float*)norm);
  } else {
    o.adam_t += 1;
    const float b1 = 0.9f, b2 = 0.999f;
    const float bc1 = 1.0f - (float)pow((double)b1, (double)o.adam_t);
    const float bc2s = (float)sqrt(1.0 - pow((double)b2, (double)o.adam_t));
    hipLaunchKernelGGL(adam_update, dim3(ceil_div(n / 4, 256)), dim3(256), 0, s, P, G, S1, S2, n / 4, o.lr, b1, b2, o.eps,
                       bc1, bc2s, (const float*)norm);
  }
}

}
}
```

### rela_amd/csrc/learner_r2d2.hip

```cpp
#include "gemm_bf16s.h"
#include "learner_common.h"

using namespace rela_amd;

namespace rela_amd {
namespace {

constexpr int kHid = 512, kGates = 2048, kFeat = 3136;
constexpr int kRecSplitF = 4;
constexpr int kRecSplitB = 8;

using TileRows = TileCfg<128, 64, 4, 2, false>;
using TileRec = TileCfg<64, 64, 2, 4, false>;
using TileWg = TileCfg<128, 64, 4, 2, true>;
using TileW32r = TileCfg<32, 64, 2, 4, true>;

struct ProbGateX : ProbBase {
  const float *a3, *wihT, *bias;
  float* gx;
  __device__ float4 loadA(int m, int k) const { return m < M ? ld4(a3 + (size_t)m * kFeat + k) : zero4(); }
  __device__ float4 loadB(int k, int n) const { return ld4(wihT + (size_t)k * kGates + n); }
  __device__ void store(int, int m, int n, float v) const { gx[(size_t)m * kGates + n] = v + bias[n]; }
};
struct ProbRecFwd : ProbBase {
  const float *h, *whhT;
  float* part;
  __device__ float4 loadA(int m, int k) const { return m < M ? ld4(h + (size_t)m * kHid + k) : zero4(); }
  __device__ float4 loadB(int k, int n) const { return ld4(whhT + (size_t)k * kGates + n); }
  __device__ void store(int z, int m, int n, float v) const { part[((size_t)z * M + m) * kGates + n] = v; }
};
struct ProbRecBwd : ProbBase {
  const float *dg, *whh;
  float* part;
  __device__ float4 loadA(int m, int k) const { return m < M ? ld4(dg + (size_t)m * kGates + k) : zero4(); }
  __device__ float4 loadB(int k, int n) const { return ld4(whh + (size_t)k * kHid + n); }
  __device__ void store(int z, int m, int n, float v) const { part[((size_t)z * M + m) * kHid + n] = v; }
};
struct ProbWhh : ProbBase {
  const float *dg, *hprev;
  float* out;
  __device__ float4 loadA(int r, int m) const { return r < K ? ld4(dg + (size_t)r * kGates + m) : zero4(); }
  __device__ float4 loadB(int r, int n) const { return r < K ? ld4(hprev + (size_t)r * kHid + n) : zero4(); }
  __device__ void store(int, int m, int n, float v) const { out[(size_t)m * kHid + n] = v; }
};
struct ProbWih : ProbBase {
  const float *dg, *a3;
  float* out;
  __device__ float4 loadA(int r, int m) const { return r < K ? ld4(dg + (size_t)r * kGates + m) : zero4(); }
  __device__ float4 loadB(int r, int n) const { return r < K ? ld4(a3 + (size_t)r * kFeat + n) : zero4(); }
  __device__ void store(int, int m, int n, float v) const {
    const int pos = n >> 6, c = n & 63;
    out[(size_t)m * kFeat + c * 49 + pos] = v;
  }
};
struct ProbIhDgrad : ProbBase {
  const float *dg, *wihp, *a3;
  float* d_a3;
  __device__ float4 loadA(int m, int k) const { return m < M ? ld4(dg + (size_t)m * kGates + k) : zero4(); }
  __device__ float4 loadB(int k, int n) const { return ld4(wihp + (size_t)k * kFeat + n); }
  __device__ void store(int, int m, int n, float v) const {
    const size_t i = (size_t)m * kFeat + n;
    d_a3[i] = a3[i] > 0.f ? v : 0.f;
  }
};
struct ProbHeadDgradSeq : ProbBase {
  const float *d_ha, *a_w, *v_w;
  float* d_o;
  int A;
  __device__ float4 loadA(int m, int k) const { return m < M ? ld4(d_ha + (size_t)m * 32 + k) : zero4(); }
  __device__ float4 loadB(int k, int n) const {
    if (k < A) return ld4(a_w + (size_t)k * kHid + n);
    if (k == 31) return ld4(v_w + n);
    return zero4();
  }
  __device__ void store(int, int m, int n, float v) const { d_o[(size_t)m * kHid + n] = v; }
};

constexpr int kPackRows = 8;
__global__ __launch_bounds__(256) void pack_lstm_learner(const float* __restrict__ wih, const float* __restrict__ whh,
                                                         const float* __restrict__ bih, const float* __restrict__ bhh,
                                                         float* __restrict__ wihT, float* __restrict__ wihp,
                                                         float* __restrict__ whhT, float* __restrict__ bsum) {
  extern __shared__ __attribute__((aligned(16))) float rows[];
  const int g0 = blockIdx.x * kPackRows, tid = threadIdx.x;
  for (int i = tid; i < kPackRows * kFeat / 4; i += 256)
    reinterpret_cast<float4*>(rows)[i] = reinterpret_cast<const float4*>(wih + (size_t)g0 * kFeat)[i];
  __syncthreads();
  if (wihp) {
    for (int i = tid; i < kPackRows * kFeat; i += 256) {
      const int r = i / kFeat, k = i - r * kFeat;
      wihp[(size_t)(g0 + r) * kFeat + k] = rows[r * kFeat + (k & 63) * 49 + (k >> 6)];
    }
  }
  for (int i = tid; i < kPackRows * kFeat; i += 256) {
    const int k = i / kPackRows, r = i - k * kPackRows;
    wihT[(size_t)k * kGates + g0 + r] = rows[r * kFeat + (k & 63) * 49 + (k >> 6)];
  }
  __syncthreads();
  for (int i = tid; i < kPackRows * kHid / 4; i += 256)
    reinterpret_cast<float4*>(rows)[i] = reinterpret_cast<const float4*>(whh + (size_t)g0 * kHid)[i];
  __syncthreads();
  for (int i = tid; i < kPackRows * kHid; i += 256) {
    const int k = i / kPackRows, r = i - k * kPackRows;
    whhT[(size_t)k * kGates + g0 + r] = rows[r * kHid + k];
  }
  if (tid < kPackRows) bsum[g0 + tid] = bih[g0 + tid] + bhh[g0 + tid];
}

__device__ __forceinline__ float sigm(float x) { return 1.0f / (1.0f + expf(-x)); }

__global__ void lstm_cell_fwd(float* __restrict__ gx, const float* __restrict__ part, int nsplit, int Bn,
                              const float* __restrict__ c_prev, float* __restrict__ c_out, float* __restrict__ h_out,
                              int save) {
  const int idx = blockIdx.x * blockDim.x + threadIdx.x;
  if (idx >= Bn * kHid) return;
  const int b = idx / kHid, u = idx - b * kHid;
  float pre[4];
#pragma unroll
  for (int q = 0; q < 4; ++q) {
    const size_t o = (size_t)b * kGates + q * kHid + u;
    float v = gx[o];
    for (int z = 0; z < nsplit; ++z) v += part[(size_t)z * Bn * kGates + o];
    pre[q] = v;
  }
  const float gi = sigm(pre[0]), gf = sigm(pre[1]), gg = tanhf(pre[2]), go = sigm(pre[3]);
  const float c = gf * c_prev[idx] + gi * gg;
  c_out[idx] = c;
  h_out[idx] = go * tanhf(c);
  if (save) {
    float* row = gx + (size_t)b * kGates + u;
    row[0] = gi, row[kHid] = gf, row[2 * kHid] = gg, row[3 * kHid] = go;
  }
}

typedef unsigned int u32x4 __attribute__((ext_vector_type(4)));
__device__ __forceinline__ __amdgpu_buffer_rsrc_t sc1_rsrc(const void* base, size_t bytes) {
  return __builtin_amdgcn_make_buffer_rsrc(const_cast<void*>(base), 0, (int)bytes, 0x00020000);
}
template <bool SC1>
__device__ __forceinline__ float4 ld4_shared(__amdgpu_buffer_rsrc_t rs, const float* base, size_t index) {
  if constexpr (SC1) {
    const u32x4 v = __builtin_amdgcn_raw_buffer_load_b128(rs, (int)(index * 4), 0, 16);
    return make_float4(__uint_as_float(v[0]), __uint_as_float(v[1]), __uint_as_float(v[2]), __uint_as_float(v[3]));
  } else {
    return *reinterpret_cast<const float4*>(base + index);
  }
}

typedef __attribute__((address_space(1))) unsigned gu32;
typedef __attribute__((address_space(1))) unsigned long long gu64;
constexpr int kRecThreads = 512;
constexpr unsigned kRecSpinLimit = 1u << 22;
struct RecNet {
  float* gx;
  const float* whhT;
  float *H, *C;
  unsigned* bar;
  int save;
};
struct ChainArgs2 {
  RecNet net[2];
  const uint8_t* term;
  unsigned* tmo;
  unsigned* bar;
  int T, Tpad, Bn, burn;
};
constexpr int kChainBlocks = 32, kChainUnits = kHid / kChainBlocks;
static_assert(kChainUnits == 16, "tile shapes below");
template <bool SC1>
__global__ __launch_bounds__(kRecThreads) void lstm_rec_chain(ChainArgs2 a) {
  __shared__ float red[8][16][65];
  __shared__ int alive;
  const int tid = threadIdx.x, wave = tid >> 6, lane = tid & 63;
  const int li = lane & 15, g = lane >> 4;
  const int chain = blockIdx.x & 7, j = blockIdx.x >> 3;
  const RecNet nt = a.net[chain >> 2];
  const int row0 = (chain & 3) * 16;
  if (row0 >= a.Bn) return;
  const int nrow = min(16, a.Bn - row0);
  float bfr[4][16];
#pragma unroll
  for (int c = 0; c < 4; ++c)
#pragma unroll
    for (int ks = 0; ks < 16; ++ks) bfr[c][ks] = nt.whhT[(size_t)(wave * 64 + 16 * g + ks) * kGates + c * kHid + 16 * j + li];
  const size_t blk = (size_t)a.Bn * kHid;
  const __amdgpu_buffer_rsrc_t rsH = sc1_rsrc(nt.H, (size_t)(a.T + 1) * blk * 4);
  const int cu = tid & 15, cr = tid >> 4;
  const bool cell = tid < 256 && cr < nrow;
  const int crow = row0 + cr;
  float c_reg = 0.f;
  if (cell) c_reg = nt.C[(size_t)crow * kHid + 16 * j + cu];
  float gpre[4];
  auto gx_fetch = [&](int t) {
    const float* grow = nt.gx + ((size_t)t * a.Bn + crow) * kGates + 16 * j + cu;
#pragma unroll
    for (int q = 0; q < 4; ++q) gpre[q] = grow[q * kHid];
  };
  if (cell) gx_fetch(0);
  unsigned* bar = a.bar + (size_t)chain * a.Tpad;
  for (int t = 0; t < a.T; ++t) {
    float4 hv[4];
    {
      const int arow = row0 + min(li, nrow - 1);
      const size_t hoff = (size_t)t * blk + (size_t)arow * kHid + wave * 64 + 16 * g;
#pragma unroll
      for (int q = 0; q < 4; ++q) hv[q] = ld4_shared<SC1>(rsH, nt.H, hoff + 4 * q);
    }
    const float av[16] = {hv[0].x, hv[0].y, hv[0].z, hv[0].w, hv[1].x, hv[1].y, hv[1].z, hv[1].w,
                          hv[2].x, hv[2].y, hv[2].z, hv[2].w, hv[3].x, hv[3].y, hv[3].z, hv[3].w};
    f32x4 acc[4];
#pragma unroll
    for (int c = 0; c < 4; ++c) {
      acc[c] = f32x4{0.f, 0.f, 0.f, 0.f};
#pragma unroll
      for (int ks = 0; ks < 16; ++ks) acc[c] = __builtin_amdgcn_mfma_f32_16x16x4f32(av[ks], bfr[c][ks], acc[c], 0, 0, 0);
    }
#pragma unroll
    for (int c = 0; c < 4; ++c)
#pragma unroll
      for (int r = 0; r < 4; ++r) red[wave][4 * g + r][c * 16 + li] = acc[c][r];
    __syncthreads();
    if (cell) {
      float pre[4];
#pragma unroll
      for (int q = 0; q < 4; ++q) {
        pre[q] = gpre[q];
#pragma unroll
        for (int w = 0; w < 8; ++w) pre[q] += red[w][cr][q * 16 + cu];
      }
      const bool zero = a.burn > 0 && t + 1 == a.burn && a.term[(size_t)(a.burn - 1) * a.Bn + crow] != 0;
      const float gi = sigm(pre[0]), gf = sigm(pre[1]), gg = tanhf(pre[2]), go = sigm(pre[3]);
      float c = gf * c_reg + gi * gg;
      float h = go * tanhf(c);
      if (zero) c = 0.f, h = 0.f;
      c_reg = c;
      const size_t o = (size_t)(t + 1) * blk + (size_t)crow * kHid + 16 * j + cu;
      __hip_atomic_store((gu32*)(nt.H + o), __float_as_uint(h), __ATOMIC_RELAXED, __HIP_MEMORY_SCOPE_AGENT);
      nt.C[o] = c;
      if (nt.save && t >= a.burn) {
        float* grow = nt.gx + ((size_t)t * a.Bn + crow) * kGates + 16 * j + cu;
        grow[0] = gi, grow[kHid] = gf, grow[2 * kHid] = gg, grow[3 * kHid] = go;
      }
    }
    if (t + 1 == a.T) break;
    asm volatile("s_waitcnt vmcnt(0)" ::: "memory");
    __syncthreads();
    if (cell) gx_fetch(t + 1);
    if (tid == 0) {
      gu32* cnt = (gu32*)(bar + t);
      __hip_atomic_fetch_add(cnt, 1u, __ATOMIC_RELAXED, __HIP_MEMORY_SCOPE_AGENT);
      bool ok = true;
      for (unsigned spins = 0; __hip_atomic_load(cnt, __ATOMIC_RELAXED, __HIP_MEMORY_SCOPE_AGENT) < (unsigned)kChainBlocks;) {
        __builtin_amdgcn_s_sleep(1);
        if (++spins > kRecSpinLimit || __hip_atomic_load((gu32*)a.tmo, __ATOMIC_RELAXED, __HIP_MEMORY_SCOPE_AGENT) != 0) {
          __hip_atomic_store((gu32*)a.tmo, (unsigned)(t + 1), __ATOMIC_RELAXED, __HIP_MEMORY_SCOPE_AGENT);
          ok = false;
          break;
        }
      }
      if constexpr (!SC1) {
        __builtin_amdgcn_fence(__ATOMIC_ACQUIRE, "agent");
        asm volatile("s_waitcnt vmcnt(0)" ::: "memory");
      }
      alive = ok ? 1 : 0;
    }
    __syncthreads();
    if (!alive) return;
  }
}

constexpr int kBpttBlocks = kHid / 16;

struct BpttArgs {
  float* ga;
  const float* d_o;
  const float* whh;
  const float* C;
  float* dc_rec;
  unsigned* bar;
  unsigned* tmo;
  int Tt, Bn, burn;
};

template <bool SC1>
__global__ __launch_bounds__(kRecThreads) void lstm_bptt_chain(BpttArgs a, int Tpad) {
  __shared__ float red[8][16][17];
  __shared__ int alive;
  const int tid = threadIdx.x, wave = tid >> 6, lane = tid & 63;
  const int li = lane & 15, g = lane >> 4, chain = blockIdx.x & 7, j = blockIdx.x >> 3;
  const int row0 = chain * 16;
  if (row0 >= a.Bn) return;
  float bfr[64];
#pragma unroll
  for (int ks = 0; ks < 64; ++ks) bfr[ks] = a.whh[(size_t)(256 * wave + 64 * g + ks) * kHid + 16 * j + li];
  const size_t blk = (size_t)a.Bn * kHid;
  const __amdgpu_buffer_rsrc_t rsG = sc1_rsrc(a.ga, (size_t)a.Tt * a.Bn * kGates * 4);
  const int r = tid >> 2, q = tid & 3, row = row0 + r;
  const bool cell = tid < 4 * 16 && row < a.Bn;
  const size_t u0 = (size_t)row * kHid + 16 * j + 4 * q;
  float dcr[4] = {0.f, 0.f, 0.f, 0.f};
  if (cell) {
    const float4 d4 = *reinterpret_cast<const float4*>(a.dc_rec + u0);
    dcr[0] = d4.x, dcr[1] = d4.y, dcr[2] = d4.z, dcr[3] = d4.w;
  }
  unsigned* bar = a.bar + (size_t)chain * Tpad;
  for (int t = a.Tt - 1; t >= 0; --t) {
    const bool rec = t + 1 < a.Tt;
    float* ga_t = a.ga + (size_t)t * a.Bn * kGates;
    if (rec) {
      f32x4 acc = f32x4{0.f, 0.f, 0.f, 0.f};
      const int arow = min(row0 + li, a.Bn - 1);
      const size_t doff = (size_t)(t + 1) * a.Bn * kGates + (size_t)arow * kGates + 256 * wave + 64 * g;
      float4 v[16];
#pragma unroll
      for (int c = 0; c < 16; ++c) v[c] = ld4_shared<SC1>(rsG, a.ga, doff + 4 * c);
#pragma unroll
      for (int c = 0; c < 16; ++c) {
        acc = __builtin_amdgcn_mfma_f32_16x16x4f32(v[c].x, bfr[4 * c], acc, 0, 0, 0);
        acc = __builtin_amdgcn_mfma_f32_16x16x4f32(v[c].y, bfr[4 * c + 1], acc, 0, 0, 0);
        acc = __builtin_amdgcn_mfma_f32_16x16x4f32(v[c].z, bfr[4 * c + 2], acc, 0, 0, 0);
        acc = __builtin_amdgcn_mfma_f32_16x16x4f32(v[c].w, bfr[4 * c + 3], acc, 0, 0, 0);
      }
#pragma unroll
      for (int rr = 0; rr < 4; ++rr) red[wave][4 * g + rr][li] = acc[rr];
    }
    __syncthreads();
    if (cell) {
      const int gs = a.burn + t;
      const float4 d_o4 = *reinterpret_cast<const float4*>(a.d_o + (size_t)t * blk + u0);
      float dh[4] = {d_o4.x, d_o4.y, d_o4.z, d_o4.w};
      if (rec) {
#pragma unroll
        for (int u = 0; u < 4; ++u)
#pragma unroll
          for (int w = 0; w < 8; ++w) dh[u] += red[w][r][4 * q + u];
      }
      float* grow = ga_t + (size_t)row * kGates + 16 * j + 4 * q;
      const float4 gi4 = *reinterpret_cast<const float4*>(grow), gf4 = *reinterpret_cast<const float4*>(grow + kHid);
      const float4 gg4 = *reinterpret_cast<const float4*>(grow + 2 * kHid), go4 = *reinterpret_cast<const float4*>(grow + 3 * kHid);
      const float4 cn4 = *reinterpret_cast<const float4*>(a.C + (size_t)(gs + 1) * blk + u0);
      const float4 cp4 = *reinterpret_cast<const float4*>(a.C + (size_t)gs * blk + u0);
      const float gi[4] = {gi4.x, gi4.y, gi4.z, gi4.w}, gf[4] = {gf4.x, gf4.y, gf4.z, gf4.w};
      const float gg[4] = {gg4.x, gg4.y, gg4.z, gg4.w}, go[4] = {go4.x, go4.y, go4.z, go4.w};
      const float cn[4] = {cn4.x, cn4.y, cn4.z, cn4.w}, cp[4] = {cp4.x, cp4.y, cp4.z, cp4.w};
      float di[4], df[4], dgg[4], dgo[4];
#pragma unroll
      for (int u = 0; u < 4; ++u) {
        const float tc = tanhf(cn[u]);
        const float dc = dcr[u] + dh[u] * go[u] * (1.0f - tc * tc);
        di[u] = dc * gg[u] * gi[u] * (1.0f - gi[u]);
        df[u] = dc * cp[u] * gf[u] * (1.0f - gf[u]);
        dgg[u] = dc * gi[u] * (1.0f - gg[u] * gg[u]);
        dgo[u] = dh[u] * tc * go[u] * (1.0f - go[u]);
        dcr[u] = dc * gf[u];
      }
      auto store_wt = [&](float* dst, const float* v) {
        gu64* p = (gu64*)dst;
        __hip_atomic_store(p, ((unsigned long long)__float_as_uint(v[1]) << 32) | __float_as_uint(v[0]),
                           __ATOMIC_RELAXED, __HIP_MEMORY_SCOPE_AGENT);
        __hip_atomic_store(p + 1, ((unsigned long long)__float_as_uint(v[3]) << 32) | __float_as_uint(v[2]),
                           __ATOMIC_RELAXED, __HIP_MEMORY_SCOPE_AGENT);
      };
      store_wt(grow, di);
      store_wt(grow + kHid, df);
      store_wt(grow + 2 * kHid, dgg);
      store_wt(grow + 3 * kHid, dgo);
    }
    if (t == 0) break;
    asm volatile("s_waitcnt vmcnt(0)" ::: "memory");
    __syncthreads();
    if (tid == 0) {
      gu32* cnt = (gu32*)(bar + t);
      __hip_atomic_fetch_add(cnt, 1u, __ATOMIC_RELAXED, __HIP_MEMORY_SCOPE_AGENT);
      bool ok = true;
      for (unsigned spins = 0; __hip_atomic_load(cnt, __ATOMIC_RELAXED, __HIP_MEMORY_SCOPE_AGENT) < (unsigned)kBpttBlocks;) {
        __builtin_amdgcn_s_sleep(1);
        if (++spins > kRecSpinLimit || __hip_atomic_load((gu32*)a.tmo, __ATOMIC_RELAXED, __HIP_MEMORY_SCOPE_AGENT) != 0) {
          __hip_atomic_store((gu32*)a.tmo, (unsigned)(1000 + t), __ATOMIC_RELAXED, __HIP_MEMORY_SCOPE_AGENT);
          ok = false;
          break;
        }
      }
      if constexpr (!SC1) {
        __builtin_amdgcn_fence(__ATOMIC_ACQUIRE, "agent");
        asm volatile("s_waitcnt vmcnt(0)" ::: "memory");
      }
      alive = ok ? 1 : 0;
    }
    __syncthreads();
    if (!alive) return;
  }
  if (cell) *reinterpret_cast<float4*>(a.dc_rec + u0) = make_float4(dcr[0], dcr[1], dcr[2], dcr[3]);
}

__global__ void zero_hidden_where_terminal(const uint8_t* __restrict__ term, int Bn, float* __restrict__ h,
                                           float* __restrict__ c) {
  const int idx = blockIdx.x * blockDim.x + threadIdx.x;
  if (idx >= Bn * kHid) return;
  if (term[idx / kHid]) h[idx] = 0.f, c[idx] = 0.f;
}

__global__ void lstm_cell_bwd(float* __restrict__ ga, const float* __restrict__ d_o, const float* __restrict__ dh_part,
                              int nsplit, int Bn, const float* __restrict__ c_now, const float* __restrict__ c_prev,
                              float* __restrict__ dc_rec) {
  const int idx = blockIdx.x * blockDim.x + threadIdx.x;
  if (idx >= Bn * kHid) return;
  const int b = idx / kHid, u = idx - b * kHid;
  float dh = d_o[idx];
  for (int z = 0; z < nsplit; ++z) dh += dh_part[(size_t)z * Bn * kHid + idx];
  float* row = ga + (size_t)b * kGates + u;
  const float gi = row[0], gf = row[kHid], gg = row[2 * kHid], go = row[3 * kHid];
  const float tc = tanhf(c_now[idx]);
  const float dc = dc_rec[idx] + dh * go * (1.0f - tc * tc);
  row[0] = dc * gg * gi * (1.0f - gi);
  row[kHid] = dc * c_prev[idx] * gf * (1.0f - gf);
  row[2 * kHid] = dc * gi * (1.0f - gg * gg);
  row[3 * kHid] = dh * tc * go * (1.0f - go);
  dc_rec[idx] = dc * gf;
}

__global__ __launch_bounds__(1024) void q_min_all(const float* __restrict__ q, int64_t n, float* __restrict__ out) {
  __shared__ float red[1024];
  float m = INFINITY;
  for (int64_t i = threadIdx.x; i < n; i += 1024) m = fminf(m, q[i]);
  red[threadIdx.x] = m;
  __syncthreads();
  for (int o = 512; o > 0; o >>= 1) {
    if ((int)threadIdx.x < o) red[threadIdx.x] = fminf(red[threadIdx.x], red[threadIdx.x + o]);
    __syncthreads();
  }
  if (threadIdx.x == 0) out[0] = red[0];
}

__global__ void seq_select(const float* __restrict__ q_on, const float* __restrict__ q_tg,
                           const float* __restrict__ legal, const int64_t* __restrict__ act,
                           const float* __restrict__ qmin, int rows, int A, float* __restrict__ qa_on,
                           float* __restrict__ qa_tg) {
  const int r = blockIdx.x * blockDim.x + threadIdx.x;
  if (r >= rows) return;
  const float mn = qmin[0];
  const float* qo = q_on + (size_t)r * A;
  const float* lg = legal + (size_t)r * A;
  int best = 0;
  float bv = -INFINITY;
  for (int j = 0; j < A; ++j) {
    const float v = (1.0f + qo[j] - mn) * lg[j];
    if (v > bv) bv = v, best = j;
  }
  qa_on[r] = qo[(int)act[r]];
  qa_tg[r] = q_tg[(size_t)r * A + best];
}

__global__ __launch_bounds__(1024) void seq_td_loss(const float* __restrict__ qa_on, const float* __restrict__ qa_tg,
                                                    const float* __restrict__ reward, const float* __restrict__ boot,
                                                    const float* __restrict__ seq_len, const float* __restrict__ w,
                                                    int Bn, int seq, int burn, int nstep, float gamma_n, float vr_eps,
                                                    float eta, float one_minus_eta, float* __restrict__ dqa,
                                                    float* __restrict__ prio, float* __restrict__ loss_seq,
                                                    float* __restrict__ loss_out) {
  __shared__ float red[1024];
  const int b = threadIdx.x;
  float lw = 0.f;
  if (b < Bn) {
    const float len = seq_len[b];
    const float inv_b = 1.0f / (float)Bn;
    float lsum = 0.f, psum = 0.f, pmax = 0.f;
    for (int i = 0; i < seq + nstep; ++i) {
      const size_t r = (size_t)i * Bn + b;
      float g = 0.f;
      if (i < seq) {
        float target;
        if (vr_eps > 0.0f)
          target = rela_vr::h(reward[r] + boot[r] * (gamma_n * rela_vr::h_inv(qa_tg[(size_t)(i + nstep) * Bn + b], vr_eps)), vr_eps);
        else
          target = reward[r] + boot[r] * (gamma_n * qa_tg[(size_t)(i + nstep) * Bn + b]);
        const bool pad = (float)i >= len - (float)burn;
        const float e = pad ? 0.f : target - qa_on[r];
        const float ae = fabsf(e);
        lsum += ae < 1.0f ? 0.5f * e * e : ae - 0.5f;
        const float pm = ((float)i < len) ? ae : 0.f;
        psum += pm;
        pmax = fmaxf(pmax, pm);
        g = pad ? 0.f : -(w[b] * fminf(fmaxf(e, -1.0f), 1.0f)) * inv_b;
      }
      dqa[r] = g;
    }
    loss_seq[b] = lsum;
    prio[b] = eta * pmax + one_minus_eta * (psum / (len - (float)burn));
    lw = lsum * w[b];
  }
  red[threadIdx.x] = lw;
  __syncthreads();
  for (int o = 512; o > 0; o >>= 1) {
    if ((int)threadIdx.x < o) red[threadIdx.x] += red[threadIdx.x + o];
    __syncthreads();
  }
  if (threadIdx.x == 0) loss_out[0] = red[0] / (float)Bn;
}

__global__ void seq_head_grad(const float* __restrict__ dqa, const int64_t* __restrict__ act,
                              const float* __restrict__ legal, int rows, int A, float* __restrict__ d_ha) {
  const int idx = blockIdx.x * blockDim.x + threadIdx.x;
  if (idx >= rows * 32) return;
  const int r = idx >> 5, k = idx & 31;
  const float g = dqa[r];
  float v = 0.f;
  if (k < A) v = legal[(size_t)r * A + k] * (g * ((k == (int)act[r] ? 1.0f : 0.0f) - 1.0f / (float)A));
  if (k == 31) v = g;
  d_ha[idx] = v;
}

}
}

struct rela_r2d2_learner {
  int device = 0;
  int A = 0, Bmax = 0, seq = 0, burn = 0, n = 0, T = 0;
  float gamma_n = 0.f, eta = 0.f, one_minus_eta = 0.f;
  float vr_eps = 0.f;
  bool loss_called = false;
  OptimState opt;
  int64_t off[15] = {0};
  float *P = nullptr, *PT = nullptr, *G = nullptr, *S1 = nullptr, *S2 = nullptr;
  rela_lstmnet *online = nullptr, *target = nullptr;
  float *w2p = nullptr, *w3p = nullptr;
  float *wihT[2] = {nullptr, nullptr}, *whhT[2] = {nullptr, nullptr}, *bsum[2] = {nullptr, nullptr};
  float* wihp = nullptr;
  float *a1 = nullptr, *a2 = nullptr, *a3 = nullptr;
  float* gxs[2] = {nullptr, nullptr};
  float*& gx = gxs[0];
  float *Hs[2] = {nullptr, nullptr}, *Cs[2] = {nullptr, nullptr};
  float* rec_part = nullptr;
  unsigned* rec_bar = nullptr;
  unsigned* rec_chain_bar = nullptr;
  bool rec_chains_fit = true;
  bool rec_persist = true;
  int precision = 0;
  uint8_t* wrec[2] = {nullptr, nullptr};
  uint8_t* wTrec = nullptr;
  uint8_t *arec = nullptr, *trec = nullptr;
  uint64_t wver[2] = {1, 1}, rec_ver[2] = {0, 0};
  uint8_t* s3rec = nullptr;
  void* wx3[2] = {nullptr, nullptr};
  uint64_t x3_ver[2] = {0, 0};
  float *ha = nullptr, *q_on = nullptr, *q_tg = nullptr;
  float *qmin = nullptr, *qa_on = nullptr, *qa_tg = nullptr, *dqa = nullptr, *d_ha = nullptr, *d_o = nullptr;
  float *dc_rec = nullptr;
  float *d_a3 = nullptr, *d_a2 = nullptr, *d_a1 = nullptr, *col = nullptr, *part = nullptr, *cpart = nullptr,
        *s32 = nullptr;
  double* npart = nullptr;
  float *norm = nullptr, *loss = nullptr, *loss_seq = nullptr;
  bool loaded = false;
  int pend_B = 0;
  const uint8_t* pend_obs = nullptr;
};

namespace {
const int64_t* seg_counts(int A, int64_t cnt[14]) {
  const int64_t c[14] = {32 * 256, 32, 64 * 512, 64, 64 * 576, 64, (int64_t)kGates * kFeat, (int64_t)kGates * kHid,
                         kGates, kGates, 512, 1, (int64_t)A * 512, A};
  for (int i = 0; i < 14; ++i) cnt[i] = c[i];
  return cnt;
}

rela_lstmnet_params lparams_at(const rela_r2d2_learner* l, float* base) {
  rela_lstmnet_params p;
  const float** f = reinterpret_cast<const float**>(&p);
  for (int i = 0; i < 14; ++i) f[i] = base + l->off[i];
  return p;
}

int repack_r2d2(rela_r2d2_learner* l, bool online, bool target, hipStream_t s) {
  static const hipError_t pack_attr = hipFuncSetAttribute(reinterpret_cast<const void*>(&pack_lstm_learner),
                                                         hipFuncAttributeMaxDynamicSharedMemorySize,
                                                         (int)(kPackRows * kFeat * sizeof(float)));
  RELA_HIP(pack_attr);
  if (online) {
    const rela_lstmnet_params p = lparams_at(l, l->P);
    int rc = rela_lstmnet_load(l->online, &p, 1, s);
    if (rc != RELA_OK) return rc;
    hipLaunchKernelGGL(permute_weights, dim3(ceil_div(64 * 512, 256)), dim3(256), 0, s, kPermConv2, p.conv2_w, l->w2p,
                       64 * 512);
    hipLaunchKernelGGL(permute_weights, dim3(ceil_div(64 * 576, 256)), dim3(256), 0, s, kPermConv3, p.conv3_w, l->w3p,
                       64 * 576);
    hipLaunchKernelGGL(pack_lstm_learner, dim3(kGates / kPackRows), dim3(256), kPackRows * kFeat * sizeof(float), s, p.w_ih, p.w_hh, p.b_ih, p.b_hh,
                       l->wihT[0], l->wihp, l->whhT[0], l->bsum[0]);
    RELA_LAUNCH_CHECK();
    l->wver[0] += 1;
  }
  if (target) {
    const rela_lstmnet_params p = lparams_at(l, l->PT);
    int rc = rela_lstmnet_load(l->target, &p, 1, s);
    if (rc != RELA_OK) return rc;
    hipLaunchKernelGGL(pack_lstm_learner, dim3(kGates / kPackRows), dim3(256), kPackRows * kFeat * sizeof(float), s, p.w_ih, p.w_hh, p.b_ih, p.b_hh,
                       l->wihT[1], (float*)nullptr, l->whhT[1], l->bsum[1]);
    RELA_LAUNCH_CHECK();
    l->wver[1] += 1;
  }
  return RELA_OK;
}

int refresh_weight_records(rela_r2d2_learner* l, int which, hipStream_t s) {
  if (l->rec_ver[which] == l->wver[which]) return RELA_OK;
  using namespace gemm16;
  ProfScope prof("learner_lstm_split_w", s);
  if (which == 0) {
    hipLaunchKernelGGL(split_rows_rec64, dim3(ceil_div((int64_t)kGates * kFeat / 8, 256)), dim3(256), 0, s,
                       (const float*)l->wihp, (int64_t)kGates, kFeat, l->wrec[0]);
    hipLaunchKernelGGL(split_rows_rec64, dim3(ceil_div((int64_t)kGates * kFeat / 8, 256)), dim3(256), 0, s,
                       (const float*)l->wihT[0], (int64_t)kFeat, kGates, l->wTrec);
  } else {
    hipLaunchKernelGGL(split_cols_rec64, dim3(kGates / 64, kFeat / 64), dim3(256), 0, s, (const float*)l->wihT[1],
                       (int64_t)kFeat, kGates, 0, l->wrec[1]);
  }
  RELA_LAUNCH_CHECK();
  l->rec_ver[which] = l->wver[which];
  return RELA_OK;
}

const char* const kTrunkNames[3] = {"learner_fwd_conv1", "learner_fwd_conv2", "learner_fwd_conv3"};

int forward_pre(rela_r2d2_learner* l, int which, int Bn, const uint8_t* obs, const float* h0, const float* c0,
                hipStream_t s) {
  const rela_lstmnet* net = which == 0 ? l->online : l->target;
  const int rowsAll = l->T * Bn;
  constexpr bool online_f32 = false;
  const bool fast_target = which == 1 && l->precision == 1;
  const bool fast_online = which == 0 && l->precision == 1 && !online_f32 && rowsAll >= 128;
  bool a3_records = false;
  int rc;
  if (fast_online) {
    rc = lstmnet_trunk_records(net, rowsAll, obs, l->a1, l->a2, l->a3, l->burn * Bn, s, kTrunkNames);
    a3_records = true;
  } else {
    const bool x3 = l->precision == 2 && l->s3rec != nullptr;
    rc = lstmnet_trunk(net, rowsAll, obs, l->a1, l->a2, l->a3, s, kTrunkNames, fast_target,
                       (fast_target || x3) ? &a3_records : nullptr, x3 ? l->s3rec : nullptr, which == 0);
  }
  if (rc != RELA_OK) return rc;
  if (l->precision == 1) {
    using namespace gemm16;
    rc = refresh_weight_records(l, which, s);
    if (rc != RELA_OK) return rc;
    const uint8_t* arec = reinterpret_cast<const uint8_t*>(l->a3);
    if (!a3_records) {
      ProfScope prof("learner_lstm_split_rows", s);
      hipLaunchKernelGGL(split_rows_rec64, dim3(ceil_div((int64_t)rowsAll * kFeat / 8, 256)), dim3(256), 0, s,
                         (const float*)l->a3, (int64_t)rowsAll, kFeat, l->arec);
      arec = l->arec;
    }
    rc = launch_rec64_nt(arec, l->wrec[which], rowsAll, kGates, kFeat / 64,
                         EpiBias{l->gxs[which], l->bsum[which], kGates}, s, "learner_lstm_gates_x");
    if (rc != RELA_OK) return rc;
    if (fast_online) {
      const size_t tr0 = (size_t)l->burn * Bn;
      rc = trunk_unsplit_rows(l->a1 + tr0 * kA1, l->a2 + tr0 * kA2, l->a3 + tr0 * kA3, rowsAll - (int)tr0, s);
      if (rc != RELA_OK) return rc;
    }
  } else if (a3_records) {
    if (l->x3_ver[which] != l->wver[which]) {
      ProfScope prof("learner_lstm_split_w", s);
      const rela_lstmnet_params p = lparams_at(l, which == 0 ? l->P : l->PT);
      rc = pack_gate_x3(p.w_ih, l->wx3[which], false, s);
      if (rc != RELA_OK) return rc;
      l->x3_ver[which] = l->wver[which];
    }
    ProfScope prof("learner_lstm_gates_x", s);
    rc = gate_x3_gemm(l->s3rec + (size_t)rowsAll * kRec2Bytes, l->wx3[which], l->bsum[which], l->gxs[which], rowsAll, s);
    if (rc != RELA_OK) return rc;
  } else {
    ProbGateX p{};
    p.M = rowsAll, p.N = kGates, p.K = kFeat;
    p.a3 = l->a3, p.wihT = l->wihT[which], p.bias = l->bsum[which], p.gx = l->gxs[which];
    launch_gemm<TileRows>(p, 1, s, "learner_lstm_gates_x");
  }
  const size_t blk = (size_t)Bn * kHid;
  RELA_HIP(dev_copy2(l->Hs[which], h0, blk * sizeof(float), l->Cs[which], c0, blk * sizeof(float), s));
  return RELA_OK;
}

int forward_rec_steps(rela_r2d2_learner* l, int which, int Bn, const uint8_t* term, bool save, hipStream_t s) {
  const int T = l->T, burn = l->burn;
  float *H = l->Hs[which], *Cc = l->Cs[which], *gx = l->gxs[which];
  const size_t blk = (size_t)Bn * kHid;
  const int cell_grid = ceil_div((int64_t)Bn * kHid, 256);
  for (int t = 0; t < T; ++t) {
    if (t == burn && burn > 0) {
      hipLaunchKernelGGL(zero_hidden_where_terminal, dim3(cell_grid), dim3(256), 0, s, term + (size_t)(burn - 1) * Bn,
                         Bn, H + t * blk, Cc + t * blk);
    }
    ProbRecFwd p{};
    p.M = Bn, p.N = kGates, p.K = kHid;
    p.h = H + t * blk, p.whhT = l->whhT[which], p.part = l->rec_part;
    launch_gemm<TileRec>(p, kRecSplitF, s, "learner_lstm_rec_fwd");
    ProfScope prof("learner_lstm_cell", s);
    hipLaunchKernelGGL(lstm_cell_fwd, dim3(cell_grid), dim3(256), 0, s, gx + (size_t)t * Bn * kGates,
                       (const float*)l->rec_part, kRecSplitF, Bn, (const float*)(Cc + t * blk), Cc + (t + 1) * blk,
                       H + (t + 1) * blk, (save && t >= burn) ? 1 : 0);
  }
  RELA_LAUNCH_CHECK();
  return RELA_OK;
}

int forward_both(rela_r2d2_learner* l, int Bn, const uint8_t* obs, const float* legal_train, const uint8_t* term,
                 const float* h0, const float* c0, hipStream_t s) {
  const int T = l->T, burn = l->burn, Tt = T - burn;
  int rc = forward_pre(l, 1, Bn, obs, h0, c0, s);
  if (rc != RELA_OK) return rc;
  rc = forward_pre(l, 0, Bn, obs, h0, c0, s);
  if (rc != RELA_OK) return rc;
  if (l->rec_persist && l->rec_chains_fit && Bn <= 64) {
    const int Tpad = (T + 3) / 4 * 4;
    RELA_HIP(hipMemsetAsync(l->rec_chain_bar, 0, sizeof(unsigned) * (size_t)(8 * Tpad), s));
    ChainArgs2 ca{};
    for (int w = 0; w < 2; ++w) {
      ca.net[w].gx = l->gxs[w], ca.net[w].whhT = l->whhT[w], ca.net[w].H = l->Hs[w], ca.net[w].C = l->Cs[w];
      ca.net[w].bar = nullptr, ca.net[w].save = w == 0 ? 1 : 0;
    }
    ca.term = term, ca.tmo = l->rec_bar, ca.bar = l->rec_chain_bar, ca.T = T, ca.Tpad = Tpad, ca.Bn = Bn, ca.burn = burn;
    ProfScope prof("learner_lstm_rec_persist", s);
    hipLaunchKernelGGL(lstm_rec_chain<true>, dim3(8 * kChainBlocks), dim3(kRecThreads), 0, s, ca);
    RELA_LAUNCH_CHECK();
  } else {
    rc = forward_rec_steps(l, 1, Bn, term, false, s);
    if (rc != RELA_OK) return rc;
    rc = forward_rec_steps(l, 0, Bn, term, true, s);
    if (rc != RELA_OK) return rc;
  }
  const size_t blk = (size_t)Bn * kHid;
  rc = lstmnet_heads(l->target, Tt * Bn, l->Hs[1] + (size_t)(burn + 1) * blk, legal_train, l->ha, l->q_tg, s,
                     "learner_fwd_heads");
  if (rc != RELA_OK) return rc;
  return lstmnet_heads(l->online, Tt * Bn, l->Hs[0] + (size_t)(burn + 1) * blk, legal_train, l->ha, l->q_on, s,
                       "learner_fwd_heads");
}
}

extern "C" int rela_r2d2_learner_create(rela_r2d2_learner** out, int num_action, int max_batch, int multi_step,
                                        float gamma, int seq_len, int burn_in, double eta, int optimizer, float lr,
                                        float eps, float grad_clip, int device) {
  RELA_CHECK(out && num_action >= 1 && num_action <= 31 && max_batch >= 1 && max_batch <= 1024 && multi_step >= 1 &&
                 seq_len >= 1 && burn_in >= 0 && (optimizer == 0 || optimizer == 1),
             RELA_EINVAL, "rela_r2d2_learner_create: bad arguments (A=%d batch=%d n=%d seq=%d burn=%d optimizer=%d)",
             num_action, max_batch, multi_step, seq_len, burn_in, optimizer);
  int ndev = 0;
  if (hipGetDeviceCount(&ndev) != hipSuccess || device < 0 || device >= ndev) {
    set_last_error("rela_r2d2_learner_create: HIP device %d not available (%d visible); there is no CPU path", device,
                   ndev);
    return RELA_ENODEV;
  }
  DeviceGuard g(device);
  auto* l = new rela_r2d2_learner();
  l->device = device;
  l->A = num_action, l->Bmax = max_batch, l->seq = seq_len, l->burn = burn_in, l->n = multi_step;
  l->T = burn_in + seq_len + multi_step;
  l->gamma_n = (float)pow((double)gamma, (double)multi_step);
  l->eta = (float)eta;
  l->one_minus_eta = (float)(1.0 - eta);
  l->opt.optimizer = optimizer, l->opt.lr = lr, l->opt.eps = eps, l->opt.clip = grad_clip;
  int64_t cnt[14];
  seg_counts(num_action, cnt);
  for (int i = 0; i < 14; ++i) l->off[i + 1] = l->off[i] + (cnt[i] + 3) / 4 * 4;
  const size_t nb = sizeof(float) * (size_t)l->off[14];
  const size_t B = (size_t)max_batch, A = (size_t)num_action, T = (size_t)l->T, Tt = T - burn_in;
  const size_t rowsAll = T * B, rowsTr = Tt * B;
  auto alloc = [&](float** p, size_t floats, bool zero) -> int {
    RELA_HIP(hipMalloc(p, sizeof(float) * floats));
    if (zero) RELA_HIP(hipMemset(*p, 0, sizeof(float) * floats));
    return RELA_OK;
  };
#define R2_ALLOC(ptr, floats, zero)               \
  do {                                            \
    int _rc = alloc(&(ptr), (floats), (zero));    \
    if (_rc != RELA_OK) return _rc;               \
  } while (0)
  R2_ALLOC(l->P, l->off[14], true);
  R2_ALLOC(l->PT, l->off[14], true);
  R2_ALLOC(l->G, l->off[14], true);
  R2_ALLOC(l->S1, l->off[14], true);
  R2_ALLOC(l->S2, l->off[14], true);
  (void)nb;
  int rc = rela_lstmnet_create(&l->online, num_action, device);
  if (rc != RELA_OK) return rc;
  rc = rela_lstmnet_create(&l->target, num_action, device);
  if (rc != RELA_OK) return rc;
  R2_ALLOC(l->w2p, 64 * 512, false);
  R2_ALLOC(l->w3p, 64 * 576, false);
  for (int w = 0; w < 2; ++w) {
    R2_ALLOC(l->wihT[w], (size_t)kGates * kFeat, false);
    R2_ALLOC(l->whhT[w], (size_t)kGates * kHid, false);
    R2_ALLOC(l->bsum[w], kGates, false);
    R2_ALLOC(l->Hs[w], (T + 1) * B * kHid, true);
    R2_ALLOC(l->Cs[w], (T + 1) * B * kHid, true);
  }
  R2_ALLOC(l->wihp, (size_t)kGates * kFeat, false);
  {
    const size_t chunks = (rowsAll + 63) / 64;
    float* tmp = nullptr;
    for (int w = 0; w < 2; ++w) {
      R2_ALLOC(tmp, (size_t)kGates * kFeat, false);
      l->wrec[w] = reinterpret_cast<uint8_t*>(tmp);
    }
    R2_ALLOC(tmp, (size_t)kGates * kFeat, false);
    l->wTrec = reinterpret_cast<uint8_t*>(tmp);
    R2_ALLOC(tmp, rowsAll * kFeat, false);
    l->arec = reinterpret_cast<uint8_t*>(tmp);
    R2_ALLOC(tmp, (size_t)(kGates + kFeat) * chunks * 64, false);
    l->trec = reinterpret_cast<uint8_t*>(tmp);
  }
  {
    float* tmp = nullptr;
    R2_ALLOC(tmp, (rowsAll * (size_t)(kRec2Bytes + kRec3Bytes) + 3) / 4, false);
    l->s3rec = reinterpret_cast<uint8_t*>(tmp);
    for (int w = 0; w < 2; ++w) {
      R2_ALLOC(tmp, ((size_t)gate_x3_packed_bytes() + 3) / 4, false);
      l->wx3[w] = tmp;
    }
  }
  R2_ALLOC(l->a1, rowsAll * kA1, false);
  R2_ALLOC(l->a2, rowsAll * kA2, false);
  R2_ALLOC(l->a3, rowsAll * kA3, false);
  R2_ALLOC(l->gxs[0], rowsAll * kGates, false);
  R2_ALLOC(l->gxs[1], rowsAll * kGates, false);
  {
    const size_t f = (size_t)kRecSplitF * B * kGates, b = (size_t)kRecSplitB * B * kHid;
    R2_ALLOC(l->rec_part, f > b ? f : b, false);
  }
  RELA_HIP(hipMalloc(&l->rec_bar, sizeof(unsigned) * (size_t)(8 + 2 * ((T + 3) / 4 * 4))));
  RELA_HIP(hipMemset(l->rec_bar, 0, sizeof(unsigned) * (size_t)(8 + 2 * ((T + 3) / 4 * 4))));
  RELA_HIP(hipMalloc(&l->rec_chain_bar, sizeof(unsigned) * (size_t)(8 * ((T + 3) / 4 * 4))));
  l->rec_persist = !(getenv("RELA_R2D2_REC") && strcmp(getenv("RELA_R2D2_REC"), "steps") == 0);
  if (l->rec_persist) {
    int cus = 0;
    RELA_HIP(hipDeviceGetAttribute(&cus, hipDeviceAttributeMultiprocessorCount, device));
    int occ_c = 0, occ_d = 0;
    if (hipOccupancyMaxActiveBlocksPerMultiprocessor(&occ_c, lstm_rec_chain<true>, kRecThreads, 0) != hipSuccess) occ_c = 0;
    if (hipOccupancyMaxActiveBlocksPerMultiprocessor(&occ_d, lstm_bptt_chain<false>, kRecThreads, 0) != hipSuccess) occ_d = 0;
    auto room = [cus](int occ) { return (int64_t)cus * (occ >= 4 ? occ - 1 : occ); };
    if (room(occ_c) < 8 * kChainBlocks || room(occ_d) < 8 * kBpttBlocks) {
      fprintf(stderr, "rela_r2d2_learner_create: %d CUs x (%d, %d) resident blocks cannot hold the persistent recurrent "
                      "grids (%d, %d): using the per-step launches\n", cus, occ_c, occ_d, 8 * kChainBlocks, 8 * kBpttBlocks);
      l->rec_chains_fit = false;
    }
  }
  R2_ALLOC(l->ha, rowsTr * 32, false);
  R2_ALLOC(l->q_on, rowsTr * A, false);
  R2_ALLOC(l->q_tg, rowsTr * A, false);
  R2_ALLOC(l->qmin, 4, false);
  R2_ALLOC(l->qa_on, rowsTr, false);
  R2_ALLOC(l->qa_tg, rowsTr, false);
  R2_ALLOC(l->dqa, rowsTr, false);
  R2_ALLOC(l->d_ha, rowsTr * 32, false);
  R2_ALLOC(l->d_o, rowsTr * kHid, false);
  R2_ALLOC(l->dc_rec, B * kHid, false);
  R2_ALLOC(l->d_a3, rowsTr * kA3, false);
  R2_ALLOC(l->d_a2, rowsTr * kA2, false);
  R2_ALLOC(l->d_a1, rowsTr * kA1, false);
  R2_ALLOC(l->col, trunk_col_floats(rowsTr), false);
  R2_ALLOC(l->part, kTrunkPartFloats, false);
  R2_ALLOC(l->cpart, (size_t)kColsumBlocks * kGates, false);
  R2_ALLOC(l->s32, 32, false);
  R2_ALLOC(l->norm, 2, true);
  R2_ALLOC(l->loss, 1, true);
  R2_ALLOC(l->loss_seq, B, true);
#undef R2_ALLOC
  RELA_HIP(hipMalloc(&l->npart, sizeof(double) * kNormBlocks));
  *out = l;
  return RELA_OK;
}

extern "C" void rela_r2d2_learner_destroy(rela_r2d2_learner* l) {
  if (!l) return;
  DeviceGuard g(l->device);
  (void)hipDeviceSynchronize();
  void* ps[] = {l->P,      l->PT,     l->G,       l->S1,      l->S2,      l->w2p,     l->w3p,   l->wihT[0], l->wihT[1],
                l->whhT[0], l->whhT[1], l->bsum[0], l->bsum[1], l->Hs[0],   l->Hs[1],   l->Cs[0], l->Cs[1],   l->wihp,
                l->a1,    l->a2,      l->a3,      l->gx,      l->rec_part, l->ha,   l->q_on,    l->q_tg,
                l->qmin,   l->qa_on,  l->qa_tg,   l->dqa,     l->d_ha,    l->d_o,     l->dc_rec, l->d_a3,   l->d_a2,
                l->d_a1,   l->col,    l->part,    l->cpart,   l->s32,     l->npart,   l->norm,  l->loss,    l->loss_seq};
  for (void* p : ps) (void)hipFree(p);
  (void)hipFree(l->rec_bar);
  (void)hipFree(l->rec_chain_bar);
  (void)hipFree(l->gxs[1]);
  (void)hipFree(l->wrec[0]);
  (void)hipFree(l->wrec[1]);
  (void)hipFree(l->wTrec);
  (void)hipFree(l->arec);
  (void)hipFree(l->s3rec);
  (void)hipFree(l->wx3[0]);
  (void)hipFree(l->wx3[1]);
  (void)hipFree(l->trec);
  rela_lstmnet_destroy(l->online);
  rela_lstmnet_destroy(l->target);
  delete l;
}

extern "C" int rela_r2d2_learner_load(rela_r2d2_learner* l, const rela_lstmnet_params* online,
                                      const rela_lstmnet_params* target, int on_device, void* stream_) {
  RELA_CHECK(l && online, RELA_EINVAL, "rela_r2d2_learner_load: bad arguments");
  hipStream_t s = (hipStream_t)stream_;
  DeviceGuard g(l->device);
  const hipMemcpyKind kind = on_device ? hipMemcpyDeviceToDevice : hipMemcpyHostToDevice;
  const float* const* fo = reinterpret_cast<const float* const*>(online);
  const float* const* ft = reinterpret_cast<const float* const*>(target ? target : online);
  int64_t cnt[14];
  seg_counts(l->A, cnt);
  for (int i = 0; i < 14; ++i) {
    RELA_CHECK(fo[i] && ft[i], RELA_EINVAL, "rela_r2d2_learner_load: parameter %d is NULL", i);
    RELA_HIP(hipMemcpyAsync(l->P + l->off[i], fo[i], sizeof(float) * cnt[i], kind, s));
    RELA_HIP(hipMemcpyAsync(l->PT + l->off[i], ft[i], sizeof(float) * cnt[i], kind, s));
  }
  if (!on_device) RELA_HIP(hipStreamSynchronize(s));
  const size_t nb = sizeof(float) * (size_t)l->off[14];
  RELA_HIP(hipMemsetAsync(l->S1, 0, nb, s));
  RELA_HIP(hipMemsetAsync(l->S2, 0, nb, s));
  l->opt.adam_t = 0;
  int rc = repack_r2d2(l, true, true, s);
  if (rc != RELA_OK) return rc;
  l->loaded = true;
  return RELA_OK;
}

extern "C" int rela_r2d2_learner_sync_target(rela_r2d2_learner* l, void* stream_) {
  RELA_CHECK(l && l->loaded, RELA_ESTATE, "rela_r2d2_learner_sync_target: parameters were never loaded");
  hipStream_t s = (hipStream_t)stream_;
  DeviceGuard g(l->device);
  RELA_HIP(hipMemcpyAsync(l->PT, l->P, sizeof(float) * (size_t)l->off[14], hipMemcpyDeviceToDevice, s));
  return repack_r2d2(l, false, true, s);
}

extern "C" int rela_r2d2_learner_params(rela_r2d2_learner* l, rela_lstmnet_params* online_out,
                                        rela_lstmnet_params* target_out) {
  RELA_CHECK(l, RELA_EINVAL, "rela_r2d2_learner_params: bad arguments");
  if (online_out) *online_out = lparams_at(l, l->P);
  if (target_out) *target_out = lparams_at(l, l->PT);
  return RELA_OK;
}

extern "C" int rela_r2d2_learner_grads(rela_r2d2_learner* l, rela_lstmnet_params* grads_out) {
  RELA_CHECK(l && grads_out, RELA_EINVAL, "rela_r2d2_learner_grads: bad arguments");
  *grads_out = lparams_at(l, l->G);
  return RELA_OK;
}

extern "C" int rela_r2d2_learner_flat(rela_r2d2_learner* l, float** params_dev, float** grads_dev, int64_t* count) {
  RELA_CHECK(l, RELA_EINVAL, "rela_r2d2_learner_flat: bad arguments");
  if (params_dev) *params_dev = l->P;
  if (grads_dev) *grads_dev = l->G;
  if (count) *count = l->off[14];
  return RELA_OK;
}

extern "C" const float* rela_r2d2_learner_stats_dev(const rela_r2d2_learner* l) { return l ? l->norm : nullptr; }

extern "C" int rela_r2d2_learner_set_value_rescale(rela_r2d2_learner* l, float eps) {
  RELA_CHECK(l && eps == eps, RELA_EINVAL, "rela_r2d2_learner_set_value_rescale: bad arguments");
  RELA_CHECK(!l->loss_called, RELA_ESTATE, "rela_r2d2_learner_set_value_rescale: call it before the first loss");
  l->vr_eps = eps > 0.f ? eps : 0.f;
  return RELA_OK;
}

extern "C" int rela_r2d2_learner_set_precision(rela_r2d2_learner* l, int mode) {
  RELA_CHECK(l && mode >= 0 && mode <= 2, RELA_EINVAL, "rela_r2d2_learner_set_precision: mode must be 0, 1 or 2");
  l->precision = mode;
  int rc = rela_lstmnet_set_precision(l->online, mode == 2 ? 2 : 0);
  if (rc != RELA_OK) return rc;
  return rela_lstmnet_set_precision(l->target, mode == 2 ? 2 : 0);
}

extern "C" int rela_r2d2_learner_check(rela_r2d2_learner* l, void* stream_) {
  RELA_CHECK(l, RELA_EINVAL, "rela_r2d2_learner_check: null learner");
  DeviceGuard g(l->device);
  RELA_HIP(hipStreamSynchronize((hipStream_t)stream_));
  unsigned tmo = 0;
  RELA_HIP(hipMemcpy(&tmo, l->rec_bar, sizeof(unsigned), hipMemcpyDeviceToHost));
  if (tmo != 0) {
    RELA_HIP(hipMemset(l->rec_bar, 0, sizeof(unsigned)));
    l->rec_persist = false;
    set_last_error("rela_r2d2_learner_check: the grid barrier of a persistent recurrent kernel timed out at step %u: the "
                   "results of that call are invalid, no optimiser update was applied since, and this learner now uses "
                   "the per-step launches", tmo - 1);
    return RELA_ESTATE;
  }
  return RELA_OK;
}

extern "C" int rela_r2d2_learner_backward(rela_r2d2_learner* l, int batch, const void* const* rows_dev,
                                          const float* weight_dev, float* priority_dev, float* loss_dev,
                                          float* loss_seq_dev, void* stream_) {
  int rc = rela_r2d2_learner_loss(l, batch, rows_dev, weight_dev, priority_dev, loss_dev, loss_seq_dev, stream_);
  if (rc != RELA_OK) return rc;
  return rela_r2d2_learner_grad(l, stream_);
}

extern "C" int rela_r2d2_learner_loss(rela_r2d2_learner* l, int batch, const void* const* rows_dev,
                                      const float* weight_dev, float* priority_dev, float* loss_dev,
                                      float* loss_seq_dev, void* stream_) {
  RELA_CHECK(l && l->loaded, RELA_ESTATE, "rela_r2d2_learner_loss: parameters were never loaded");
  RELA_CHECK(batch >= 1 && batch <= l->Bmax && rows_dev && weight_dev && priority_dev, RELA_EINVAL,
             "rela_r2d2_learner_loss: bad arguments (batch %d, max %d)", batch, l->Bmax);
  hipStream_t s = (hipStream_t)stream_;
  DeviceGuard g(l->device);
  l->pend_B = 0;
  l->loss_called = true;
  const int Bn = batch, A = l->A, T = l->T, burn = l->burn, Tt = T - burn, rowsTr = Tt * Bn;
  const uint8_t* obs = static_cast<const uint8_t*>(rows_dev[0]);
  const float* legal = static_cast<const float*>(rows_dev[2]);
  const int64_t* act = static_cast<const int64_t*>(rows_dev[3]);
  const float* reward = static_cast<const float*>(rows_dev[4]);
  const uint8_t* term = static_cast<const uint8_t*>(rows_dev[5]);
  const float* boot = static_cast<const float*>(rows_dev[6]);
  const float* h0 = static_cast<const float*>(rows_dev[7]);
  const float* c0 = static_cast<const float*>(rows_dev[8]);
  const float* seq_len = static_cast<const float*>(rows_dev[9]);
  RELA_CHECK(obs && legal && act && reward && term && boot && h0 && c0 && seq_len, RELA_EINVAL,
             "rela_r2d2_learner_loss: a batch field is NULL");
  const size_t tr0 = (size_t)burn * Bn;
  const float* legal_tr = legal + tr0 * A;
  const int64_t* act_tr = act + tr0;
  int rc = forward_both(l, Bn, obs, legal_tr, term, h0, c0, s);
  if (rc != RELA_OK) return rc;
  {
    ProfScope prof("learner_seq_td", s);
    hipLaunchKernelGGL(q_min_all, dim3(1), dim3(1024), 0, s, (const float*)l->q_on, (int64_t)rowsTr * A, l->qmin);
    hipLaunchKernelGGL(seq_select, dim3(ceil_div(rowsTr, 256)), dim3(256), 0, s, (const float*)l->q_on,
                       (const float*)l->q_tg, legal_tr, act_tr, (const float*)l->qmin, rowsTr, A, l->qa_on, l->qa_tg);
    hipLaunchKernelGGL(seq_td_loss, dim3(1), dim3(1024), 0, s, (const float*)l->qa_on, (const float*)l->qa_tg,
                       reward + tr0, boot + tr0, seq_len, weight_dev, Bn, l->seq, burn, l->n, l->gamma_n, l->vr_eps, l->eta,
                       l->one_minus_eta, l->dqa, priority_dev, l->loss_seq, l->loss);
    hipLaunchKernelGGL(seq_head_grad, dim3(ceil_div((int64_t)rowsTr * 32, 256)), dim3(256), 0, s, (const float*)l->dqa,
                       act_tr, legal_tr, rowsTr, A, l->d_ha);
  }
  if (loss_dev) RELA_HIP(hipMemcpyAsync(loss_dev, l->loss, sizeof(float), hipMemcpyDeviceToDevice, s));
  if (loss_seq_dev)
    RELA_HIP(hipMemcpyAsync(loss_seq_dev, l->loss_seq, sizeof(float) * Bn, hipMemcpyDeviceToDevice, s));
  RELA_LAUNCH_CHECK();
  l->pend_B = Bn;
  l->pend_obs = obs;
  return RELA_OK;
}

extern "C" int rela_r2d2_learner_grad(rela_r2d2_learner* l, void* stream_) {
  RELA_CHECK(l && l->loaded && l->pend_B > 0, RELA_ESTATE, "rela_r2d2_learner_grad: no rela_r2d2_learner_loss to differentiate");
  hipStream_t s = (hipStream_t)stream_;
  DeviceGuard g(l->device);
  const int Bn = l->pend_B, A = l->A, T = l->T, burn = l->burn, Tt = T - burn, rowsTr = Tt * Bn;
  const uint8_t* obs = l->pend_obs;
  const size_t tr0 = (size_t)burn * Bn;
  l->pend_B = 0;

  const rela_lstmnet_params P = lparams_at(l, l->P);
  float* Gm[14];
  for (int i = 0; i < 14; ++i) Gm[i] = l->G + l->off[i];
  const size_t blk = (size_t)Bn * kHid;
  float *H = l->Hs[0], *Cc = l->Cs[0];
  const float* o_tr = H + (size_t)(burn + 1) * blk;
  {
    ProbHeadDgradSeq p{};
    p.M = rowsTr, p.N = kHid, p.K = 32;
    p.d_ha = l->d_ha, p.a_w = P.a_w, p.v_w = P.v_w, p.d_o = l->d_o, p.A = A;
    launch_gemm<TileRows>(p, 1, s, "learner_dgrad_heads");
  }
  if (rowsTr >= 1024) {
    constexpr int kSplitHeads = 32;
    static_assert((size_t)kSplitHeads * 32 * 512 <= kTrunkPartFloats, "part size");
    ProbHeadWgradPart p{};
    p.M = 32, p.N = kHid, p.K = rowsTr;
    p.d_ha = l->d_ha, p.h = o_tr, p.part = l->part;
    launch_gemm<TileW32r>(p, kSplitHeads, s, "learner_wgrad_heads");
    hipLaunchKernelGGL(head_wgrad_reduce, dim3(ceil_div(32 * 512, 256)), dim3(256), 0, s, (const float*)l->part,
                       kSplitHeads, A, Gm[12], Gm[10]);
  } else {
    ProbHeadWgrad p{};
    p.M = 32, p.N = kHid, p.K = rowsTr;
    p.d_ha = l->d_ha, p.h = o_tr, p.g_a_w = Gm[12], p.g_v_w = Gm[10], p.A = A;
    launch_gemm<TileW32r>(p, 1, s, "learner_wgrad_heads");
  }
  colsum_launch(l->d_ha, rowsTr, 32, l->cpart, l->s32, s);
  hipLaunchKernelGGL(head_bias_grad, dim3(1), dim3(32), 0, s, (const float*)l->s32, A, Gm[13], Gm[11]);
  RELA_HIP(hipMemsetAsync(l->dc_rec, 0, blk * sizeof(float), s));
  const int cell_grid = ceil_div((int64_t)Bn * kHid, 256);
  float* ga_tr = l->gx + tr0 * kGates;
  if (l->rec_persist && l->rec_chains_fit && Bn <= 128 && Tt <= l->T) {
    const int Tpad_c = (l->T + 3) / 4 * 4;
    RELA_HIP(hipMemsetAsync(l->rec_chain_bar, 0, sizeof(unsigned) * (size_t)(8 * Tpad_c), s));
    BpttArgs ba{};
    ba.ga = ga_tr, ba.d_o = l->d_o, ba.whh = P.w_hh, ba.C = Cc, ba.dc_rec = l->dc_rec;
    ba.bar = l->rec_chain_bar, ba.tmo = l->rec_bar, ba.Tt = Tt, ba.Bn = Bn, ba.burn = burn;
    ProfScope prof("learner_lstm_bptt_persist", s);
    hipLaunchKernelGGL(lstm_bptt_chain<false>, dim3(8 * kBpttBlocks), dim3(kRecThreads), 0, s, ba, Tpad_c);
  } else
  for (int t = Tt - 1; t >= 0; --t) {
    const int gs = burn + t;
    {
      ProfScope prof("learner_lstm_cell_bwd", s);
      hipLaunchKernelGGL(lstm_cell_bwd, dim3(cell_grid), dim3(256), 0, s, ga_tr + (size_t)t * Bn * kGates,
                         (const float*)(l->d_o + (size_t)t * blk), (const float*)l->rec_part,
                         t == Tt - 1 ? 0 : kRecSplitB, Bn, (const float*)(Cc + (size_t)(gs + 1) * blk),
                         (const float*)(Cc + (size_t)gs * blk), l->dc_rec);
    }
    if (t > 0) {
      ProbRecBwd p{};
      p.M = Bn, p.N = kHid, p.K = kGates;
      p.dg = ga_tr + (size_t)t * Bn * kGates, p.whh = P.w_hh, p.part = l->rec_part;
      launch_gemm<TileRec>(p, kRecSplitB, s, "learner_lstm_rec_bwd");
    }
  }
  const float* DG = ga_tr;
  const float* hprev = H + (size_t)burn * blk;
  const float* a3_tr = l->a3 + tr0 * kA3;
  if (l->precision != 1) {
    ProbWhh p{};
    p.M = kGates, p.N = kHid, p.K = rowsTr;
    p.dg = DG, p.hprev = hprev, p.out = Gm[7];
    launch_gemm<TileWg>(p, 1, s, "learner_wgrad_lstm_hh");
  }
  if (l->precision == 1) {
    using namespace gemm16;
    const int chunks = ceil_div(rowsTr, 64);
    uint8_t* dgT = l->trec;
    uint8_t* a3T = l->trec + (size_t)kGates * chunks * REC;
    {
      ProfScope prof("learner_lstm_split_cols", s);
      hipLaunchKernelGGL(split_cols_rec64, dim3(kGates / 64, chunks), dim3(256), 0, s, DG, (int64_t)rowsTr, kGates, 0, dgT);
      hipLaunchKernelGGL(split_cols_rec64, dim3(kFeat / 64, chunks), dim3(256), 0, s, a3_tr, (int64_t)rowsTr, kFeat, 1, a3T);
    }
    int rc = launch_rec64_nt(dgT, a3T, kGates, kFeat, chunks, EpiPlain{Gm[6], kFeat}, s, "learner_wgrad_lstm_ih");
    if (rc != RELA_OK) return rc;
    {
      ProfScope prof("learner_lstm_split_cols", s);
      hipLaunchKernelGGL(split_cols_rec64, dim3(kHid / 64, chunks), dim3(256), 0, s, hprev, (int64_t)rowsTr, kHid, 0, a3T);
    }
    rc = launch_rec64_nt(dgT, a3T, kGates, kHid, chunks, EpiPlain{Gm[7], kHid}, s, "learner_wgrad_lstm_hh");
    if (rc != RELA_OK) return rc;
  } else {
    ProbWih p{};
    p.M = kGates, p.N = kFeat, p.K = rowsTr;
    p.dg = DG, p.a3 = a3_tr, p.out = Gm[6];
    launch_gemm<TileWg>(p, 1, s, "learner_wgrad_lstm_ih");
  }
  colsum_launch(DG, rowsTr, kGates, l->cpart, Gm[8], s);
  RELA_HIP(hipMemcpyAsync(Gm[9], Gm[8], sizeof(float) * kGates, hipMemcpyDeviceToDevice, s));
  if (l->precision == 1) {
    using namespace gemm16;
    {
      ProfScope prof("learner_lstm_split_rows", s);
      hipLaunchKernelGGL(split_rows_rec64, dim3(ceil_div((int64_t)rowsTr * kGates / 8, 256)), dim3(256), 0, s, DG,
                         (int64_t)rowsTr, kGates, l->arec);
    }
    int rc = launch_rec64_nt(l->arec, l->wTrec, rowsTr, kFeat, kGates / 64, EpiReluMask{l->d_a3, a3_tr, kFeat}, s,
                             "learner_dgrad_lstm_ih");
    if (rc != RELA_OK) return rc;
  } else {
    ProbIhDgrad p{};
    p.M = rowsTr, p.N = kFeat, p.K = kGates;
    p.dg = DG, p.wihp = l->wihp, p.a3 = a3_tr, p.d_a3 = l->d_a3;
    launch_gemm<TileRows>(p, 1, s, "learner_dgrad_lstm_ih");
  }
  {
    TrunkBwd t{};
    t.Bn = rowsTr, t.obs = obs + tr0 * 28224, t.a1 = l->a1 + tr0 * kA1, t.a2 = l->a2 + tr0 * kA2, t.d_a3 = l->d_a3;
    t.d_a2 = l->d_a2, t.d_a1 = l->d_a1, t.col = l->col, t.part = l->part, t.cpart = l->cpart;
    t.w2p = l->w2p, t.w3p = l->w3p;
    t.g_c1w = Gm[0], t.g_c1b = Gm[1], t.g_c2w = Gm[2], t.g_c2b = Gm[3], t.g_c3w = Gm[4], t.g_c3b = Gm[5];
    t.fast = l->precision == 1;
    trunk_backward(t, s);
  }
  RELA_LAUNCH_CHECK();
  return RELA_OK;
}

extern "C" int rela_r2d2_learner_apply(rela_r2d2_learner* l, void* stream_) {
  RELA_CHECK(l && l->loaded, RELA_ESTATE, "rela_r2d2_learner_apply: parameters were never loaded");
  hipStream_t s = (hipStream_t)stream_;
  DeviceGuard g(l->device);
  optimizer_apply(l->opt, l->P, l->G, l->S1, l->S2, l->off[14], l->npart, l->norm, s, l->rec_bar);
  RELA_LAUNCH_CHECK();
  return repack_r2d2(l, true, false, s);
}
```

Baseline: 3.372 million env-steps/s.

## Fuse col2im into implicit-GEMM conv data gradients and single-part conv1 B operand

Replaces the conv3/conv2 data-gradient GEMM-plus-col2im scatter with implicit-GEMM (gather) formulations that fold the ReLU mask into the store. This drops the large col buffer and its write/read traffic, and adds a chunk-folding accumulator. Separately, the emulated conv1 weight gradient treats the uint8 observation operand as exactly representable in one bf16 part, cutting MFMAs and LDS. The change also caps trunk frames per step to keep the grid y extent valid.

Result: faster. 3.424 million env-steps/s, median of 6 (+1.5%).

```diff
diff --git a/rela_amd/csrc/gemm_bf16x3.h b/rela_amd/csrc/gemm_bf16x3.h
--- a/rela_amd/csrc/gemm_bf16x3.h
+++ b/rela_amd/csrc/gemm_bf16x3.h
@@ -49,6 +49,7 @@
 template <int BM_, int BN_, int WM_, int WN_, bool AMC_, int PARTS_ = 2>
 struct TileCfg {
   static constexpr int BM = BM_, BN = BN_, WM = WM_, WN = WN_, PARTS = PARTS_;
+  static constexpr int BPARTS = PARTS;
   static constexpr bool AMC = AMC_;
   static_assert(PARTS == 2 || PARTS == 3, "two or three bf16 parts per operand");
   static_assert(WM * WN == 8, "8 wavefronts per block");
@@ -64,6 +65,13 @@
   static constexpr int A_V4 = BM * BK / 4, B_V4 = BN * BK / 4;
   static constexpr int A_IT = (A_V4 + kT - 1) / kT, B_IT = (B_V4 + kT - 1) / kT;
 };
+template <class Base>
+struct SinglePartB : Base {
+  static_assert(Base::PARTS == 3, "the one-part B operand goes with a three-part A");
+  static constexpr int BPARTS = 1;
+  static constexpr int BUF = Base::PARTS * Base::A_HALF + Base::B_HALF;
+  static constexpr int LDS_BYTES = 2 * BUF;
+};
 
 struct GridMap {
   int gx, gy, gz;
@@ -154,8 +162,8 @@
       else split4(rb[S][j], hi, lo);
       const int off = krow(kr) * T::LDB + q * 8;
       *reinterpret_cast<uint2*>(bb + off) = hi;
-      if constexpr (T::PARTS == 3) *reinterpret_cast<uint2*>(bb + T::B_HALF + off) = mid;
-      *reinterpret_cast<uint2*>(bb + (T::PARTS - 1) * T::B_HALF + off) = lo;
+      if constexpr (T::BPARTS == 3) *reinterpret_cast<uint2*>(bb + T::B_HALF + off) = mid;
+      if constexpr (T::BPARTS > 1) *reinterpret_cast<uint2*>(bb + (T::BPARTS - 1) * T::B_HALF + off) = lo;
     }
   };
 
@@ -197,12 +205,12 @@
     if (cur + D < c1) gload(cur + D, cs);
     const uint8_t* base = smem + buf * T::BUF;
     const uint8_t* bb = base + T::PARTS * T::A_HALF;
-    bf16x8 bp[T::TN][T::PARTS];
+    bf16x8 bp[T::TN][T::BPARTS];
 #pragma unroll
     for (int u = 0; u < T::TN; ++u) {
       const int col0 = (wn * T::TN + u) * 16;
 #pragma unroll
-      for (int q = 0; q < T::PARTS; ++q) bp[u][q] = frag_tr(bb + q * T::B_HALF, T::LDB, col0);
+      for (int q = 0; q < T::BPARTS; ++q) bp[u][q] = frag_tr(bb + q * T::B_HALF, T::LDB, col0);
     }
 #pragma unroll
     for (int t = 0; t < T::TM; ++t) {
@@ -218,6 +226,10 @@
         if constexpr (T::PARTS == 2) {
           acc[t][u] = __builtin_amdgcn_mfma_f32_16x16x32_bf16(ap[1], bp[u][0], acc[t][u], 0, 0, 0);
           acc[t][u] = __builtin_amdgcn_mfma_f32_16x16x32_bf16(ap[0], bp[u][1], acc[t][u], 0, 0, 0);
+          acc[t][u] = __builtin_amdgcn_mfma_f32_16x16x32_bf16(ap[0], bp[u][0], acc[t][u], 0, 0, 0);
+        } else if constexpr (T::BPARTS == 1) {
+          accs[t][u] = __builtin_amdgcn_mfma_f32_16x16x32_bf16(ap[2], bp[u][0], accs[t][u], 0, 0, 0);
+          accs[t][u] = __builtin_amdgcn_mfma_f32_16x16x32_bf16(ap[1], bp[u][0], accs[t][u], 0, 0, 0);
           acc[t][u] = __builtin_amdgcn_mfma_f32_16x16x32_bf16(ap[0], bp[u][0], acc[t][u], 0, 0, 0);
         } else {
           accs[t][u] = __builtin_amdgcn_mfma_f32_16x16x32_bf16(ap[2], bp[u][0], accs[t][u], 0, 0, 0);
diff --git a/rela_amd/csrc/gemm_lds.h b/rela_amd/csrc/gemm_lds.h
--- a/rela_amd/csrc/gemm_lds.h
+++ b/rela_amd/csrc/gemm_lds.h
@@ -1,5 +1,7 @@
 #pragma once
 #include <hip/hip_runtime.h>
+
+#include <type_traits>
 
 #include "common.h"
 #include "prof.h"
@@ -27,6 +29,15 @@
   static constexpr int B_FLOATS = BK * LDB;
   static constexpr int A_V4 = BM * BK / 4, B_V4 = BN * BK / 4;
   static constexpr int A_IT = (A_V4 + kLT - 1) / kLT, B_IT = (B_V4 + kLT - 1) / kLT;
+};
+
+template <class P, class = void>
+struct fold_chunks {
+  static constexpr int value = 0;
+};
+template <class P>
+struct fold_chunks<P, std::void_t<decltype(P::kFoldChunks)>> {
+  static constexpr int value = P::kFoldChunks;
 };
 
 template <class T, class P>
@@ -98,6 +109,14 @@
   for (int t = 0; t < T::TM; ++t)
 #pragma unroll
     for (int u = 0; u < T::TN; ++u) acc[t][u] = f32x4{0.f, 0.f, 0.f, 0.f};
+  constexpr int FOLD = fold_chunks<P>::value;
+  f32x4 tot[FOLD ? T::TM : 1][FOLD ? T::TN : 1];
+  if constexpr (FOLD > 0) {
+#pragma unroll
+    for (int t = 0; t < T::TM; ++t)
+#pragma unroll
+      for (int u = 0; u < T::TN; ++u) tot[t][u] = f32x4{0.f, 0.f, 0.f, 0.f};
+  }
 
   if (c0 < c1) {
     gload(c0);
@@ -122,6 +141,17 @@
 #pragma unroll
         for (int u = 0; u < T::TN; ++u) acc[t][u] = __builtin_amdgcn_mfma_f32_16x16x4f32(a[t], b[u], acc[t][u], 0, 0, 0);
     }
+    if constexpr (FOLD > 0) {
+      if ((ch - c0 + 1) % FOLD == 0) {
+#pragma unroll
+        for (int t = 0; t < T::TM; ++t)
+#pragma unroll
+          for (int u = 0; u < T::TN; ++u) {
+            tot[t][u] += acc[t][u];
+            acc[t][u] = f32x4{0.f, 0.f, 0.f, 0.f};
+          }
+      }
+    }
     if (ch + 1 < c1) sstore(buf ^ 1);
     __syncthreads();
   }
@@ -134,7 +164,10 @@
       for (int r = 0; r < 4; ++r) {
         const int m = m0 + (wm * T::TM + t) * 16 + kk * 4 + r;
         const int n = n0 + (wn * T::TN + u) * 16 + li;
-        if (m < p.M && n < p.N) p.store(blockIdx.z, m, n, acc[t][u][r]);
+        if (m < p.M && n < p.N) {
+          if constexpr (FOLD > 0) p.store(blockIdx.z, m, n, tot[t][u][r]);
+          else p.store(blockIdx.z, m, n, acc[t][u][r]);
+        }
       }
 }
 
diff --git a/rela_amd/csrc/learner.hip b/rela_amd/csrc/learner.hip
--- a/rela_amd/csrc/learner.hip
+++ b/rela_amd/csrc/learner.hip
@@ -19,7 +19,6 @@
   int64_t ws_bytes = 0;
   float *q = nullptr;
   float *td = nullptr, *d_ha = nullptr, *d_h = nullptr, *d_a3 = nullptr, *d_a2 = nullptr, *d_a1 = nullptr;
-  float *col = nullptr;
   float *part = nullptr;
   float *cpart = nullptr;
   float *s32 = nullptr;
@@ -65,7 +64,7 @@
 extern "C" int rela_apex_learner_create(rela_apex_learner** out, int num_action, int max_batch, int multi_step,
                                         float gamma, int optimizer, float lr, float eps, float grad_clip,
                                         int device) {
-  RELA_CHECK(out && num_action >= 1 && num_action <= 31 && max_batch >= 1 && multi_step >= 1 &&
+  RELA_CHECK(out && num_action >= 1 && num_action <= 31 && max_batch >= 1 && max_batch <= kTrunkMaxFrames && multi_step >= 1 &&
                  (optimizer == 0 || optimizer == 1),
              RELA_EINVAL, "rela_apex_learner_create: bad arguments (A=%d batch=%d n=%d optimizer=%d)", num_action,
              max_batch, multi_step, optimizer);
@@ -121,7 +120,6 @@
   RELA_HIP(hipMalloc(&l->d_a3, sizeof(float) * B * kA3));
   RELA_HIP(hipMalloc(&l->d_a2, sizeof(float) * B * kA2));
   RELA_HIP(hipMalloc(&l->d_a1, sizeof(float) * B * kA1));
-  RELA_HIP(hipMalloc(&l->col, sizeof(float) * trunk_col_floats(B)));
   RELA_HIP(hipMalloc(&l->part, sizeof(float) * kTrunkPartFloats));
   RELA_HIP(hipMalloc(&l->cpart, sizeof(float) * kColsumBlocks * (32 + 512 + 64 + 64 + 32)));
   RELA_HIP(hipMalloc(&l->s32, sizeof(float) * 32));
@@ -146,7 +144,7 @@
   DeviceGuard g(l->device);
   (void)hipDeviceSynchronize();
   void* ps[] = {l->P,  l->PT,   l->G,    l->S1,   l->S2,   l->w2p, l->w3p,  l->wfcp,  l->ws_on, l->ws_tmp, l->q,
-                l->td, l->d_ha, l->d_h,  l->d_a3, l->d_a2, l->d_a1, l->col, l->part,  l->cpart, l->s32,    l->npart,
+                l->td, l->d_ha, l->d_h,  l->d_a3, l->d_a2, l->d_a1, l->part,  l->cpart, l->s32,    l->npart,
                 l->norm, l->loss, l->part_side, l->cpart_side, l->frag2, l->frag3};
   for (void* p : ps) (void)hipFree(p);
   for (hipEvent_t e : l->ev)
@@ -388,7 +386,7 @@
   {
     TrunkBwd t{};
     t.Bn = Bn, t.obs = obs, t.a1 = w.a1, t.a2 = w.a2, t.d_a3 = l->d_a3, t.d_a2 = l->d_a2, t.d_a1 = l->d_a1;
-    t.col = l->col, t.part = l->part, t.cpart = l->cpart, t.w2p = l->w2p, t.w3p = l->w3p;
+    t.part = l->part, t.cpart = l->cpart, t.w2p = l->w2p, t.w3p = l->w3p;
     t.g_c1w = Gm[0], t.g_c1b = Gm[1], t.g_c2w = Gm[2], t.g_c2b = Gm[3], t.g_c3w = Gm[4], t.g_c3b = Gm[5];
     t.fast = rela_ffnet_precision(l->online) == 1;
     t.emu = g6;
@@ -431,7 +429,7 @@
                                          const float* a1, const float* a2, const float* d_a3, const float* conv2_w,
                                          const float* conv3_w, float* g_c1w, float* g_c1b, float* g_c2w, float* g_c2b,
                                          float* g_c3w, float* g_c3b, float* d_a2, float* d_a1, void* stream_) {
-  RELA_CHECK(frames >= 1 && frames <= 65536 && mode >= 0 && mode <= 2 && (lanes == 0 || lanes == 1), RELA_EINVAL,
+  RELA_CHECK(frames >= 1 && frames <= kTrunkMaxFrames && mode >= 0 && mode <= 2 && (lanes == 0 || lanes == 1), RELA_EINVAL,
              "rela_debug_trunk_backward: bad arguments (frames %d, mode %d, lanes %d)", frames, mode, lanes);
   RELA_CHECK(obs && a1 && a2 && d_a3 && conv2_w && conv3_w && g_c1w && g_c1b && g_c2w && g_c2b && g_c3w && g_c3b && d_a2 &&
                  d_a1,
@@ -450,7 +448,6 @@
   t.g_c1w = g_c1w, t.g_c1b = g_c1b, t.g_c2w = g_c2w, t.g_c2b = g_c2b, t.g_c3w = g_c3w, t.g_c3b = g_c3b;
   t.fast = mode == 1;
   if (fast_wgrad_min_frames > 0) t.fast_wgrad_min_frames = fast_wgrad_min_frames;
-  RELA_HIP(sc.alloc(&t.col, sizeof(float) * trunk_col_floats((size_t)frames)));
   RELA_HIP(sc.alloc(&t.part, sizeof(float) * kTrunkPartFloats));
   RELA_HIP(sc.alloc(&t.cpart, cpart_bytes));
   t.emu = mode == 2;
diff --git a/rela_amd/csrc/learner_common.h b/rela_amd/csrc/learner_common.h
--- a/rela_amd/csrc/learner_common.h
+++ b/rela_amd/csrc/learner_common.h
@@ -23,6 +23,8 @@
 using TileWfc = TileCfg<128, 64, 4, 2, true>;
 using TileW64 = TileCfg<64, 64, 2, 4, true>;
 using TileW32 = TileCfg<32, 64, 2, 4, true>;
+using TileDgrad3 = TileCfg<64, 64, 2, 4, false>;
+using TileDgrad2 = TileCfg<64, 32, 4, 2, false>;
 using Tile3Dgrad = gemm3::TileCfg<128, 64, 4, 2, false>;
 using Tile3Wfc = gemm3::TileCfg<128, 64, 4, 2, true>;
 using Tile3W64 = gemm3::TileCfg<64, 64, 2, 4, true>;
@@ -32,6 +34,7 @@
 using Tile6Wfc = gemm3::TileCfg<128, 64, 4, 2, true, 3>;
 using Tile6W64 = gemm3::TileCfg<64, 64, 2, 4, true, 3>;
 using Tile6W32 = gemm3::TileCfg<32, 64, 2, 4, true, 3>;
+using Tile6W32U8 = gemm3::SinglePartB<Tile6W32>;
 
 
 struct ProbHeadDgrad : ProbBase {
@@ -104,12 +107,52 @@
   }
 };
 
-struct ProbConvDgrad : ProbBase {
-  const float *d_out, *wp;
-  float* col;
-  __device__ float4 loadA(int m, int k) const { return m < M ? ld4(d_out + (size_t)m * 64 + k) : zero4(); }
-  __device__ float4 loadB(int k, int n) const { return ld4(wp + (size_t)k * N + n); }
-  __device__ void store(int, int m, int n, float v) const { col[(size_t)m * N + n] = v; }
+struct ProbDgrad3 : ProbBase {
+  static constexpr int kFoldChunks = 2;
+  const float *d_out, *wp, *a2;
+  float* d_a2;
+  __device__ float4 loadA(int m, int k) const {
+    if (m >= M) return zero4();
+    const int b = m / 81, pix = m - b * 81;
+    const int y = pix / 9, x = pix - y * 9;
+    const int tap = k >> 6, oc = k & 63;
+    const int kh = tap / 3, kw = tap - kh * 3;
+    const int oy = y - kh, ox = x - kw;
+    if ((unsigned)oy >= 7u || (unsigned)ox >= 7u) return zero4();
+    return ld4(d_out + ((size_t)b * 49 + oy * 7 + ox) * 64 + oc);
+  }
+  __device__ float4 loadB(int k, int n) const { return ld4(wp + (size_t)(k & 63) * 576 + (k >> 6) * 64 + n); }
+  __device__ void store(int, int m, int n, float v) const {
+    const size_t i = (size_t)m * 64 + n;
+    d_a2[i] = a2[i] > 0.f ? v : 0.f;
+  }
+};
+
+struct ProbDgrad2 : ProbBase {
+  static constexpr int kFoldChunks = 2;
+  const float *d_out, *wp, *a1;
+  float* d_a1;
+  __device__ float4 loadA(int m, int k) const {
+    if (m >= M) return zero4();
+    const int b = m / 100, pix = m - b * 100;
+    const int yh = pix / 10, xh = pix - yh * 10;
+    const int t = k >> 6, oc = k & 63;
+    const int oy = yh - (t >> 1), ox = xh - (t & 1);
+    if ((unsigned)oy >= 9u || (unsigned)ox >= 9u) return zero4();
+    return ld4(d_out + ((size_t)b * 81 + oy * 9 + ox) * 64 + oc);
+  }
+  __device__ float4 loadB(int k, int n) const {
+    const int cls = n >> 5, t = k >> 6;
+    const int kh = (t & 2) + (cls >> 1), kw = 2 * (t & 1) + (cls & 1);
+    return ld4(wp + (size_t)(k & 63) * 512 + (kh * 4 + kw) * 32 + (n & 31));
+  }
+  __device__ void store(int, int m, int n, float v) const {
+    const int cls = n >> 5;
+    const int b = m / 100, pix = m - b * 100;
+    const int yh = pix / 10, xh = pix - yh * 10;
+    const size_t i = ((size_t)b * 400 + (2 * yh + (cls >> 1)) * 20 + 2 * xh + (cls & 1)) * 32 + (n & 31);
+    d_a1[i] = a1[i] > 0.f ? v : 0.f;
+  }
 };
 
 template <int OC, int CIN, int KH, int KW, int STRIDE, int OH, int OW, int IH, int IW>
@@ -147,50 +190,6 @@
   __device__ void store(int z, int m, int n, float v) const { part[((size_t)z * M + m) * N + n] = v; }
 };
 
-
-__global__ void col2im3(const float* __restrict__ col, const float* __restrict__ a2, float* __restrict__ d_a2,
-                        int Bn) {
-  const int idx = blockIdx.x * blockDim.x + threadIdx.x;
-  if (idx >= Bn * 81 * 16) return;
-  const int c4 = idx & 15, pix = idx >> 4;
-  const int x = pix % 9, y = (pix / 9) % 9, b = pix / 81;
-  float4 s = zero4();
-  for (int kh = 0; kh < 3; ++kh) {
-    const int oy = y - kh;
-    if (oy < 0 || oy >= 7) continue;
-    for (int kw = 0; kw < 3; ++kw) {
-      const int ox = x - kw;
-      if (ox < 0 || ox >= 7) continue;
-      const float4 v = ld4(col + ((size_t)b * 49 + oy * 7 + ox) * 576 + (kh * 3 + kw) * 64 + c4 * 4);
-      s.x += v.x, s.y += v.y, s.z += v.z, s.w += v.w;
-    }
-  }
-  const float4 a = ld4(a2 + (size_t)pix * 64 + c4 * 4);
-  *reinterpret_cast<float4*>(d_a2 + (size_t)pix * 64 + c4 * 4) =
-      make_float4(a.x > 0.f ? s.x : 0.f, a.y > 0.f ? s.y : 0.f, a.z > 0.f ? s.z : 0.f, a.w > 0.f ? s.w : 0.f);
-}
-
-__global__ void col2im2(const float* __restrict__ col, const float* __restrict__ a1, float* __restrict__ d_a1,
-                        int Bn) {
-  const int idx = blockIdx.x * blockDim.x + threadIdx.x;
-  if (idx >= Bn * 400 * 8) return;
-  const int c4 = idx & 7, pix = idx >> 3;
-  const int x = pix % 20, y = (pix / 20) % 20, b = pix / 400;
-  float4 s = zero4();
-  for (int kh = 0; kh < 4; ++kh) {
-    const int ty = y - kh;
-    if (ty < 0 || (ty & 1) || ty > 16) continue;
-    for (int kw = 0; kw < 4; ++kw) {
-      const int tx = x - kw;
-      if (tx < 0 || (tx & 1) || tx > 16) continue;
-      const float4 v = ld4(col + ((size_t)b * 81 + (ty >> 1) * 9 + (tx >> 1)) * 512 + (kh * 4 + kw) * 32 + c4 * 4);
-      s.x += v.x, s.y += v.y, s.z += v.z, s.w += v.w;
-    }
-  }
-  const float4 a = ld4(a1 + (size_t)pix * 32 + c4 * 4);
-  *reinterpret_cast<float4*>(d_a1 + (size_t)pix * 32 + c4 * 4) =
-      make_float4(a.x > 0.f ? s.x : 0.f, a.y > 0.f ? s.y : 0.f, a.z > 0.f ? s.z : 0.f, a.w > 0.f ? s.w : 0.f);
-}
 
 enum { kRedConv1 = 0, kRedConv2 = 1, kRedConv3 = 2 };
 __global__ void reduce_splits(const float* __restrict__ part, int splits, int M, int N, int mode,
@@ -506,16 +505,17 @@
                   kTrunkPartFloats >= (size_t)w2fast::kMaxBlocks * 64 * 512,
               "part size");
 static_assert(kSplitW3 * 64 * 576 >= kSplitW2 * 64 * 512 && kSplitW3 * 64 * 576 >= kSplitW1 * 32 * 256, "part size");
-inline size_t trunk_col_floats(size_t frames) { return frames * (size_t)(81 * 512 > 49 * 576 ? 81 * 512 : 49 * 576); }
 
 constexpr int kFastWgradMinFrames = 2048;
+constexpr int kTrunkMaxFrames = 32768;
+static_assert(((size_t)kTrunkMaxFrames * 100 + TileDgrad2::BM - 1) / TileDgrad2::BM <= 65535 &&
+                  ((size_t)kTrunkMaxFrames * 81 + TileDgrad3::BM - 1) / TileDgrad3::BM <= 65535, "grid y extent of the data gradients");
 struct TrunkBwd {
   int Bn;
   const uint8_t* obs;
   const float *a1, *a2;
   const float* d_a3;
   float *d_a2, *d_a1;
-  float* col;
   float* part;
   float* cpart;
   const float *w2p, *w3p;
@@ -590,13 +590,10 @@
     ProfScope prof("learner_dgrad_conv3", s);
     (void)dgfast::launch_conv3(t.d_a3, t.w3p, t.a2, t.d_a2, Bn, t.part, s, t.frag3);
   } else {
-    ProbConvDgrad p{};
-    p.M = Bn * 49, p.N = 576, p.K = 64;
-    p.d_out = t.d_a3, p.wp = t.w3p, p.col = t.col;
-    launch_gemm<TileDgrad>(p, 1, s, "learner_dgrad_conv3");
-    ProfScope prof("learner_col2im", s);
-    hipLaunchKernelGGL(col2im3, dim3(ceil_div((int64_t)Bn * 81 * 16, 256)), dim3(256), 0, s, (const float*)t.col, t.a2,
-                       t.d_a2, Bn);
+    ProbDgrad3 p{};
+    p.M = Bn * 81, p.N = 64, p.K = 576;
+    p.d_out = t.d_a3, p.wp = t.w3p, p.a2 = t.a2, p.d_a2 = t.d_a2;
+    launch_gemm<TileDgrad3>(p, 1, s, "learner_dgrad_conv3");
   }
   if (lanes) lane_dep(t.ev_da2, s, sw);
   if (fast23) {
@@ -629,13 +626,10 @@
     ProfScope prof("learner_dgrad_conv2", s);
     (void)dgfast::launch_conv2(t.d_a2, t.w2p, t.a1, t.d_a1, Bn, t.part, s, t.frag2);
   } else {
-    ProbConvDgrad p{};
-    p.M = Bn * 81, p.N = 512, p.K = 64;
-    p.d_out = t.d_a2, p.wp = t.w2p, p.col = t.col;
-    launch_gemm<TileDgrad>(p, 1, s, "learner_dgrad_conv2");
-    ProfScope prof("learner_col2im", s);
-    hipLaunchKernelGGL(col2im2, dim3(ceil_div((int64_t)Bn * 400 * 8, 256)), dim3(256), 0, s, (const float*)t.col, t.a1,
-                       t.d_a1, Bn);
+    ProbDgrad2 p{};
+    p.M = Bn * 100, p.N = 4 * 32, p.K = 256;
+    p.d_out = t.d_a2, p.wp = t.w2p, p.a1 = t.a1, p.d_a1 = t.d_a1;
+    launch_gemm<TileDgrad2>(p, 1, s, "learner_dgrad_conv2");
   }
   if (t.fast) {
     int blocks = 0;
@@ -649,9 +643,10 @@
     ProbW1 p{};
     p.M = 32, p.N = 256, p.K = Bn * 400;
     p.d_out = t.d_a1, p.obs = t.obs, p.part = t.part;
-    if (t.emu) (void)gemm3::launch_gemm<Tile6W32>(p, kSplitW1, s, "learner_wgrad_conv1");
-    else launch_gemm<TileW32>(p, kSplitW1, s, "learner_wgrad_conv1");
-    hipLaunchKernelGGL(reduce_splits, dim3(ceil_div(32 * 256, 256)), dim3(256), 0, s, (const float*)t.part, kSplitW1, 32,
+    const int split1 = kSplitW1;
+    if (t.emu) (void)gemm3::launch_gemm<Tile6W32U8>(p, split1, s, "learner_wgrad_conv1");
+    else launch_gemm<TileW32>(p, split1, s, "learner_wgrad_conv1");
+    hipLaunchKernelGGL(reduce_splits, dim3(ceil_div(32 * 256, 256)), dim3(256), 0, s, (const float*)t.part, split1, 32,
                        256, kRedConv1, t.g_c1w);
   }
   jobs.add(t.d_a1, (int64_t)Bn * 400, 32, t.g_c1b);
diff --git a/rela_amd/csrc/learner_r2d2.hip b/rela_amd/csrc/learner_r2d2.hip
--- a/rela_amd/csrc/learner_r2d2.hip
+++ b/rela_amd/csrc/learner_r2d2.hip
@@ -546,7 +546,7 @@
   float *ha = nullptr, *q_on = nullptr, *q_tg = nullptr;
   float *qmin = nullptr, *qa_on = nullptr, *qa_tg = nullptr, *dqa = nullptr, *d_ha = nullptr, *d_o = nullptr;
   float *dc_rec = nullptr;
-  float *d_a3 = nullptr, *d_a2 = nullptr, *d_a1 = nullptr, *col = nullptr, *part = nullptr, *cpart = nullptr,
+  float *d_a3 = nullptr, *d_a2 = nullptr, *d_a1 = nullptr, *part = nullptr, *cpart = nullptr,
         *s32 = nullptr;
   double* npart = nullptr;
   float *norm = nullptr, *loss = nullptr, *loss_seq = nullptr;
@@ -764,6 +764,12 @@
   const size_t nb = sizeof(float) * (size_t)l->off[14];
   const size_t B = (size_t)max_batch, A = (size_t)num_action, T = (size_t)l->T, Tt = T - burn_in;
   const size_t rowsAll = T * B, rowsTr = Tt * B;
+  if (rowsTr > (size_t)kTrunkMaxFrames) {
+    delete l;
+    set_last_error("rela_r2d2_learner_create: %zu training frames per step, the trunk's backward pass takes %d", rowsTr,
+                   kTrunkMaxFrames);
+    return RELA_EINVAL;
+  }
   auto alloc = [&](float** p, size_t floats, bool zero) -> int {
     RELA_HIP(hipMalloc(p, sizeof(float) * floats));
     if (zero) RELA_HIP(hipMemset(*p, 0, sizeof(float) * floats));
@@ -856,7 +862,6 @@
   R2_ALLOC(l->d_a3, rowsTr * kA3, false);
   R2_ALLOC(l->d_a2, rowsTr * kA2, false);
   R2_ALLOC(l->d_a1, rowsTr * kA1, false);
-  R2_ALLOC(l->col, trunk_col_floats(rowsTr), false);
   R2_ALLOC(l->part, kTrunkPartFloats, false);
   R2_ALLOC(l->cpart, (size_t)kColsumBlocks * kGates, false);
   R2_ALLOC(l->s32, 32, false);
@@ -877,7 +882,7 @@
                 l->whhT[0], l->whhT[1], l->bsum[0], l->bsum[1], l->Hs[0],   l->Hs[1],   l->Cs[0], l->Cs[1],   l->wihp,
                 l->a1,    l->a2,      l->a3,      l->gx,      l->rec_part, l->ha,   l->q_on,    l->q_tg,
                 l->qmin,   l->qa_on,  l->qa_tg,   l->dqa,     l->d_ha,    l->d_o,     l->dc_rec, l->d_a3,   l->d_a2,
-                l->d_a1,   l->col,    l->part,    l->cpart,   l->s32,     l->npart,   l->norm,  l->loss,    l->loss_seq};
+                l->d_a1,   l->part,    l->cpart,   l->s32,     l->npart,   l->norm,  l->loss,    l->loss_seq};
   for (void* p : ps) (void)hipFree(p);
   (void)hipFree(l->rec_bar);
   (void)hipFree(l->rec_chain_bar);
@@ -1160,7 +1165,7 @@
   {
     TrunkBwd t{};
     t.Bn = rowsTr, t.obs = obs + tr0 * 28224, t.a1 = l->a1 + tr0 * kA1, t.a2 = l->a2 + tr0 * kA2, t.d_a3 = l->d_a3;
-    t.d_a2 = l->d_a2, t.d_a1 = l->d_a1, t.col = l->col, t.part = l->part, t.cpart = l->cpart;
+    t.d_a2 = l->d_a2, t.d_a1 = l->d_a1, t.part = l->part, t.cpart = l->cpart;
     t.w2p = l->w2p, t.w3p = l->w3p;
     t.g_c1w = Gm[0], t.g_c1b = Gm[1], t.g_c2w = Gm[2], t.g_c2b = Gm[3], t.g_c3w = Gm[4], t.g_c3b = Gm[5];
     t.fast = l->precision == 1;
```
